# fuxiao0719/PanopticNeRF

Hardware: AMD Instinct MI355X
Metric: Msamples/sec (coarse+fine), KITTI-360 1408x376 (higher is better)
Workload: dtype bf16

## Files before the change

include/pnr.h:

```cpp
#ifndef PNR_H
#define PNR_H
#include <stdint.h>

#ifdef __cplusplus
extern "C" {
#endif

#define PNR_OK 0
#define PNR_EINVAL (-1)
#define PNR_EHIP (-2)
#define PNR_ENODEV (-3)

#define PNR_PREC_BF16 0
#define PNR_PREC_FP32 1

int pnr_version(void);
const char* pnr_last_error(void);
int pnr_device_check(int dev, char* buf_host, int buflen);

int pnr_stratified(const float* rays, int64_t n_rays, int n_samples, int lindisp,
                   const float* t_rand, float* z_out, void* stream);

int pnr_points(const float* rays, const float* z, int64_t n_rays, int n_samples, float* pts_out,
               void* stream);

int pnr_embed(const float* x, int64_t n, int L, float* out, void* stream);

typedef struct pnr_mlp_desc {
    int32_t D, W, skip;
    int32_t xyz_L, dir_L;
    int32_t n_sem, n_inst, head_W;
    int32_t precision;
    int32_t plan;
    int32_t head_tap;
    int32_t head_depth;
    int32_t schedule;
    int32_t clk_probe[2];
    int32_t flags;
} pnr_mlp_desc;

#define PNR_MLP_SOFTMAX 1
#define PNR_MLP_WG_CAP(n) (((n) & 0x1FF) << 16)
#define PNR_MLP_TRACE 0x7A00

typedef struct pnr_mlp_params_host {
    const float* const* pts_w; const float* const* pts_b;
    const float* alpha_w; const float* alpha_b;
    const float* feature_w; const float* feature_b;
    const float* views_w; const float* views_b;
    const float* rgb_w; const float* rgb_b;
    const float* sem0_w; const float* sem0_b; const float* sem1_w; const float* sem1_b;
    const float* inst0_w; const float* inst0_b; const float* inst1_w; const float* inst1_b;
} pnr_mlp_params_host;

int64_t pnr_mlp_packed_bytes(const pnr_mlp_desc* desc);
int pnr_mlp_pack(const pnr_mlp_desc* desc, const pnr_mlp_params_host* params, void* packed_host);

int64_t pnr_mlp_pack_workspace_bytes(const pnr_mlp_desc* desc, int backward);
int pnr_mlp_pack_device(const pnr_mlp_desc* desc, const pnr_mlp_params_host* params_dev, int backward,
                        void* workspace, void* packed, void* stream);
int pnr_mlp_repack_device(const pnr_mlp_desc* desc, const pnr_mlp_params_host* params_dev, int backward,
                          void* workspace, void* packed, void* stream);

int pnr_mlp_forward(const pnr_mlp_desc* desc, const void* packed, const float* rays, const float* z,
                    int64_t n_rays, int n_samples, float* raw, int64_t raw_stride_s,
                    int64_t raw_stride_c, void* stream);

int pnr_mlp_fused_plan(const pnr_mlp_desc* desc);
int64_t pnr_mlp_forward_composite_workspace_bytes(const pnr_mlp_desc* desc, int64_t n_rays, int n_samples, int want_weights);
int pnr_mlp_forward_composite(const pnr_mlp_desc* desc, const void* packed, const float* rays, const float* z,
                              int64_t n_rays, int n_samples, const int32_t* label_sem, const int32_t* label_inst,
                              int white_bkgd, float* rgb, float* depth, float* acc, float* weights, float* sem,
                              float* inst, float* fix_sem, float* fix_inst, void* workspace, void* stream);

int pnr_mlp_forward_tiles(const pnr_mlp_desc* desc, const void* packed, const float* rays, const float* z, int64_t n_rays,
                          int n_samples, void* workspace, void* stream);
int pnr_composite_combine(const pnr_mlp_desc* desc, const void* workspace, const float* z, int64_t n_rays, int n_samples,
                          const int32_t* label_sem, const int32_t* label_inst, int white_bkgd, float* rgb, float* depth,
                          float* acc, float* weights, float* sem, float* inst, float* fix_sem, float* fix_inst, void* stream);

int pnr_mlp_query(const pnr_mlp_desc* desc, const void* packed, const float* points, int64_t n_points,
                  float* sigma, int32_t* sem_label, int32_t* inst_label, int32_t* panoptic, const int32_t* is_thing,
                  float* sem_logits, float* inst_logits, int64_t logit_stride, void* stream);
int pnr_mlp_query_supported(const pnr_mlp_desc* desc);

int pnr_mlp_train_layout(const pnr_mlp_desc* desc, int64_t n_samples, int64_t* acts_off_host ,
                         int64_t* dys_off_host );
int pnr_mlp_forward_train(const pnr_mlp_desc* desc, const void* packed, const float* rays, const float* z,
                          int64_t n_rays, int n_samples, float* raw, int64_t raw_stride_s,
                          int64_t raw_stride_c, void* acts, void* stream);
int64_t pnr_mlp_bwd_packed_bytes(const pnr_mlp_desc* desc);
int pnr_mlp_pack_bwd(const pnr_mlp_desc* desc, const pnr_mlp_params_host* params, void* packed_host);
int pnr_mlp_backward(const pnr_mlp_desc* desc, const void* packed_bwd, const float* d_raw, const void* acts,
                     void* dys, int64_t n_rays, int n_samples, void* stream);

int64_t pnr_mlp_wgrad_workspace_bytes(const pnr_mlp_desc* desc, int64_t n_samples);
int pnr_mlp_wgrad(const pnr_mlp_desc* desc, const void* acts, const void* dys, int64_t n_samples,
                  const pnr_mlp_params_host* grads_dev, void* workspace, void* stream);

int64_t pnr_mlp_fp32_acts_floats(const pnr_mlp_desc* desc, int64_t n_samples);
int64_t pnr_mlp_backward_fp32_workspace_bytes(const pnr_mlp_desc* desc, int64_t n_samples);
int pnr_mlp_forward_train_fp32(const pnr_mlp_desc* desc, const pnr_mlp_params_host* params_dev, const float* rays,
                               const float* z, int64_t n_rays, int n_samples, float* raw, int64_t raw_stride_s,
                               int64_t raw_stride_c, float* acts, void* stream);
int pnr_mlp_backward_fp32(const pnr_mlp_desc* desc, const pnr_mlp_params_host* params_dev, const float* d_raw,
                          int64_t d_raw_stride_c, const float* acts, int64_t n_rays, int n_samples,
                          const pnr_mlp_params_host* grads_dev, void* workspace, void* stream);

int pnr_composite(const float* raw, int64_t raw_stride_s, int64_t raw_stride_c, const float* z,
                  const float* rays, const float* noise, const int32_t* label_sem,
                  const int32_t* label_inst, int64_t n_rays, int n_samples, int n_sem, int n_inst,
                  int sem_mode, int white_bkgd, float* rgb, float* depth, float* acc, float* weights,
                  float* sem, float* inst, float* fix_sem, float* fix_inst, void* stream);

int pnr_composite_backward(const float* raw, int64_t raw_stride_c, const float* z, const float* rays,
                           const float* noise, int64_t n_rays, int n_samples, int n_sem, int n_inst,
                           const float* g_rgb, const float* g_depth, const float* g_acc, const float* g_sem,
                           const float* g_inst, const float* g_weights, float* d_raw, void* stream);

int pnr_composite_backward2(const float* raw, int64_t raw_stride_c, const float* z, const float* rays,
                            const float* noise, int64_t n_rays, int n_samples, int n_sem, int n_inst,
                            const float* g_rgb, const float* g_depth, const float* g_acc, const float* g_sem,
                            const float* g_inst, const float* g_weights, const int32_t* label_sem,
                            const int32_t* label_inst, const float* g_fix_sem, const float* g_fix_inst,
                            const float* ce_sem, const float* ce_inst, float* d_raw, void* stream);
int pnr_composite_backward3(const float* raw, int64_t raw_stride_c, const float* z, const float* rays,
                            const float* noise, int64_t n_rays, int n_samples, int n_sem, int n_inst, int sem_mode,
                            const float* g_rgb, const float* g_depth, const float* g_acc, const float* g_sem,
                            const float* g_inst, const float* g_weights, const int32_t* label_sem,
                            const int32_t* label_inst, const float* g_fix_sem, const float* g_fix_inst,
                            const float* ce_sem, const float* ce_inst, float* d_raw, void* stream);

typedef struct pnr_loss_cfg {
    float w_rgb, w_depth, w_sem, w_fix_sem, w_inst, w_fix_inst;
    int32_t depth_l2;
    float fix_eps;
    int32_t maps_are_prob;
} pnr_loss_cfg;
int64_t pnr_losses_workspace_bytes(int64_t n_rays);
int pnr_losses(const pnr_loss_cfg* cfg, int64_t n_rays, int n_sem, int n_inst, const float* rgb, const float* depth,
               const float* sem, const float* fix_sem, const float* inst, const float* fix_inst, const float* rgb_gt,
               const float* depth_gt, const int32_t* sem_gt, const int32_t* inst_gt, float* losses_out, float* g_rgb,
               float* g_depth, float* g_sem, float* g_fix_sem, float* g_inst, float* g_fix_inst, void* workspace, void* stream);

int64_t pnr_ce3d_workspace_bytes(int64_t n_samples);
int pnr_ce3d(const float* raw, int64_t raw_stride_c, int first_channel, int n_classes, const int32_t* label,
             int64_t n_samples, float* out2, void* workspace, void* stream);

int pnr_gen_rays(const float* intr4_host, const float* c2w12_host, int width, int height, float near_, float far_,
                 const int32_t* pix, int64_t n_rays, float* rays, void* stream);

#define PNR_FISHEYE_NEWTON_STEPS 8
#define PNR_CAMERA_PINHOLE 0
#define PNR_CAMERA_FISHEYE 1

int pnr_gen_rays_fisheye(const float* cam7_host, const float* c2w12_host, int width, int height, float near_, float far_,
                         const int32_t* pix, int64_t n_rays, float* rays, uint8_t* valid, void* stream);

int pnr_project_points(int model, const float* cam_host, const float* w2c12_host, int width, int height, const float* points,
                       int64_t n, float* uv, float* range, uint8_t* valid, void* stream);

int pnr_panoptic_labels(const float* sem, const float* inst, const int32_t* is_thing, int64_t n_rays, int n_sem, int n_inst,
// ... 60 lines not shown
```

panopticnerf_amd/_lib.py:

```python
import ctypes
import os

_HERE = os.path.dirname(os.path.abspath(__file__))
LIB_PATH = os.environ.get("PNR_LIB_PATH") or os.path.join(_HERE, "libpnr.so")

c_f = ctypes.c_void_p
c_i64 = ctypes.c_int64
c_int = ctypes.c_int

PREC_BF16, PREC_FP32 = 0, 1
MLP_SOFTMAX, MLP_TRACE = 1, 0x7A00
CAMERA_PINHOLE, CAMERA_FISHEYE = 0, 1


class LossCfg(ctypes.Structure):
    _fields_ = [("w_rgb", ctypes.c_float), ("w_depth", ctypes.c_float), ("w_sem", ctypes.c_float),
                ("w_fix_sem", ctypes.c_float), ("w_inst", ctypes.c_float), ("w_fix_inst", ctypes.c_float),
                ("depth_l2", ctypes.c_int32), ("fix_eps", ctypes.c_float), ("maps_are_prob", ctypes.c_int32)]


class MlpDesc(ctypes.Structure):
    _fields_ = [("D", ctypes.c_int32), ("W", ctypes.c_int32), ("skip", ctypes.c_int32),
                ("xyz_L", ctypes.c_int32), ("dir_L", ctypes.c_int32),
                ("n_sem", ctypes.c_int32), ("n_inst", ctypes.c_int32), ("head_W", ctypes.c_int32),
                ("precision", ctypes.c_int32), ("plan", ctypes.c_int32), ("head_tap", ctypes.c_int32),
                ("head_depth", ctypes.c_int32), ("schedule", ctypes.c_int32), ("clk_probe", ctypes.c_int32 * 2), ("flags", ctypes.c_int32)]


class RngDesc(ctypes.Structure):
    _fields_ = [("call", ctypes.c_void_p), ("ray_base", ctypes.c_int64), ("tag", ctypes.c_int32), ("scale", ctypes.c_float)]


_fp = ctypes.POINTER(ctypes.c_float)
_fpp = ctypes.POINTER(_fp)


class MlpParamsHost(ctypes.Structure):
    _fields_ = [("pts_w", _fpp), ("pts_b", _fpp),
                ("alpha_w", _fp), ("alpha_b", _fp), ("feature_w", _fp), ("feature_b", _fp),
                ("views_w", _fp), ("views_b", _fp), ("rgb_w", _fp), ("rgb_b", _fp),
                ("sem0_w", _fp), ("sem0_b", _fp), ("sem1_w", _fp), ("sem1_b", _fp),
                ("inst0_w", _fp), ("inst0_b", _fp), ("inst1_w", _fp), ("inst1_b", _fp)]


SIGNATURES = {
    "pnr_version": (c_int, []),
    "pnr_last_error": (ctypes.c_char_p, []),
    "pnr_device_check": (c_int, [c_int, ctypes.c_char_p, c_int]),
    "pnr_stratified": (c_int, [c_f, c_i64, c_int, c_int, c_f, c_f, c_f]),
    "pnr_points": (c_int, [c_f, c_f, c_i64, c_int, c_f, c_f]),
    "pnr_embed": (c_int, [c_f, c_i64, c_int, c_f, c_f]),
    "pnr_mlp_packed_bytes": (c_i64, [ctypes.POINTER(MlpDesc)]),
    "pnr_mlp_pack": (c_int, [ctypes.POINTER(MlpDesc), ctypes.POINTER(MlpParamsHost), ctypes.c_void_p]),
    "pnr_mlp_pack_workspace_bytes": (c_i64, [ctypes.POINTER(MlpDesc), c_int]),
    "pnr_mlp_pack_device": (c_int, [ctypes.POINTER(MlpDesc), ctypes.POINTER(MlpParamsHost), c_int, c_f, c_f, c_f]),
    "pnr_mlp_repack_device": (c_int, [ctypes.POINTER(MlpDesc), ctypes.POINTER(MlpParamsHost), c_int, c_f, c_f, c_f]),
    "pnr_mlp_forward": (c_int, [ctypes.POINTER(MlpDesc), c_f, c_f, c_f, c_i64, c_int, c_f, c_i64, c_i64, c_f]),
    "pnr_mlp_train_layout": (c_int, [ctypes.POINTER(MlpDesc), c_i64, ctypes.POINTER(c_i64), ctypes.POINTER(c_i64)]),
    "pnr_mlp_forward_train": (c_int, [ctypes.POINTER(MlpDesc), c_f, c_f, c_f, c_i64, c_int, c_f, c_i64, c_i64, c_f, c_f]),
    "pnr_mlp_bwd_packed_bytes": (c_i64, [ctypes.POINTER(MlpDesc)]),
    "pnr_mlp_pack_bwd": (c_int, [ctypes.POINTER(MlpDesc), ctypes.POINTER(MlpParamsHost), ctypes.c_void_p]),
    "pnr_mlp_backward": (c_int, [ctypes.POINTER(MlpDesc), c_f, c_f, c_f, c_f, c_i64, c_int, c_f]),
    "pnr_mlp_wgrad_workspace_bytes": (c_i64, [ctypes.POINTER(MlpDesc), c_i64]),
    "pnr_mlp_wgrad": (c_int, [ctypes.POINTER(MlpDesc), c_f, c_f, c_i64, ctypes.POINTER(MlpParamsHost), c_f, c_f]),
    "pnr_mlp_fp32_acts_floats": (c_i64, [ctypes.POINTER(MlpDesc), c_i64]),
    "pnr_mlp_backward_fp32_workspace_bytes": (c_i64, [ctypes.POINTER(MlpDesc), c_i64]),
    "pnr_mlp_forward_train_fp32": (c_int, [ctypes.POINTER(MlpDesc), ctypes.POINTER(MlpParamsHost), c_f, c_f, c_i64, c_int, c_f, c_i64,
                                           c_i64, c_f, c_f]),
    "pnr_mlp_backward_fp32": (c_int, [ctypes.POINTER(MlpDesc), ctypes.POINTER(MlpParamsHost), c_f, c_i64, c_f, c_i64, c_int,
                                      ctypes.POINTER(MlpParamsHost), c_f, c_f]),
    "pnr_mlp_fused_plan": (c_int, [ctypes.POINTER(MlpDesc)]),
    "pnr_mlp_forward_composite_workspace_bytes": (c_i64, [ctypes.POINTER(MlpDesc), c_i64, c_int, c_int]),
    "pnr_mlp_forward_composite": (c_int, [ctypes.POINTER(MlpDesc), c_f, c_f, c_f, c_i64, c_int, c_f, c_f, c_int,
                                          c_f, c_f, c_f, c_f, c_f, c_f, c_f, c_f, c_f, c_f]),
    "pnr_composite": (c_int, [c_f, c_i64, c_i64, c_f, c_f, c_f, c_f, c_f, c_i64, c_int, c_int, c_int, c_int,
                              c_int, c_f, c_f, c_f, c_f, c_f, c_f, c_f, c_f, c_f]),
    "pnr_composite_backward": (c_int, [c_f, c_i64, c_f, c_f, c_f, c_i64, c_int, c_int, c_int,
                                       c_f, c_f, c_f, c_f, c_f, c_f, c_f, c_f]),
    "pnr_composite_backward2": (c_int, [c_f, c_i64, c_f, c_f, c_f, c_i64, c_int, c_int, c_int,
                                        c_f, c_f, c_f, c_f, c_f, c_f, c_f, c_f, c_f, c_f, c_f, c_f, c_f, c_f]),
    "pnr_composite_backward3": (c_int, [c_f, c_i64, c_f, c_f, c_f, c_i64, c_int, c_int, c_int, c_int,
                                        c_f, c_f, c_f, c_f, c_f, c_f, c_f, c_f, c_f, c_f, c_f, c_f, c_f, c_f]),
    "pnr_losses_workspace_bytes": (c_i64, [c_i64]),
    "pnr_losses": (c_int, [ctypes.POINTER(LossCfg), c_i64, c_int, c_int] + [c_f] * 19),
    "pnr_ce3d_workspace_bytes": (c_i64, [c_i64]),
    "pnr_ce3d": (c_int, [c_f, c_i64, c_int, c_int, c_f, c_i64, c_f, c_f, c_f]),
    "pnr_gen_rays": (c_int, [ctypes.POINTER(ctypes.c_float), ctypes.POINTER(ctypes.c_float), c_int, c_int, ctypes.c_float,
                             ctypes.c_float, c_f, c_i64, c_f, c_f]),
    "pnr_gen_rays_fisheye": (c_int, [ctypes.POINTER(ctypes.c_float), ctypes.POINTER(ctypes.c_float), c_int, c_int, ctypes.c_float,
                                     ctypes.c_float, c_f, c_i64, c_f, c_f, c_f]),
    "pnr_project_points": (c_int, [c_int, ctypes.POINTER(ctypes.c_float), ctypes.POINTER(ctypes.c_float), c_int, c_int, c_f, c_i64,
                                   c_f, c_f, c_f, c_f]),
    "pnr_panoptic_labels": (c_int, [c_f, c_f, c_f, c_i64, c_int, c_int, c_f, c_f, c_f, c_f]),
    "pnr_confusion": (c_int, [c_f, c_f, c_i64, c_int, c_f, c_f]),
    "pnr_sample_pdf": (c_int, [c_f, c_f, c_f, c_i64, c_int, c_int, c_f, c_f, c_f, c_f]),
    "pnr_bbox_hits": (c_int, [c_f, c_i64, c_f, c_int, c_int, c_f, c_f, c_f, c_f]),
    "pnr_restrict_rays": (c_int, [c_f, c_i64, c_f, c_f, c_int, c_f, c_f]),
    "pnr_sample_labels": (c_int, [c_f, c_i64, c_int, c_f, c_f, c_f, c_int, c_f, c_f, c_f, c_f]),
    "pnr_ray_setup": (c_int, [c_f, c_i64, c_f, c_int, c_int, c_f, c_int, c_int, c_f, c_int, c_f, c_f, c_f, c_f, c_f, c_f, c_f]),
    "pnr_sample_pdf_labels": (c_int, [c_f, c_f, c_f, c_i64, c_int, c_int, c_f, c_f, c_f, c_f, c_int, c_f, c_f, c_f, c_f]),
    "pnr_mlp_forward_tiles": (c_int, [ctypes.POINTER(MlpDesc), c_f, c_f, c_f, c_i64, c_int, c_f, c_f]),
    "pnr_rng_begin": (c_int, [c_f, c_f, c_f]),
    "pnr_rng_fill": (c_int, [ctypes.POINTER(RngDesc), c_i64, c_int, c_int, c_f, c_f]),
    "pnr_stratified_rng": (c_int, [c_f, c_i64, c_int, c_int, ctypes.POINTER(RngDesc), c_f, c_f]),
    "pnr_ray_setup_rng": (c_int, [c_f, c_i64, c_f, c_int, c_int, c_f, c_int, c_int, ctypes.POINTER(RngDesc), c_int, c_f, c_f, c_f, c_f,
                                  c_f, c_f, c_f]),
    "pnr_sample_pdf_rng": (c_int, [c_f, c_f, ctypes.POINTER(RngDesc), c_i64, c_int, c_int, c_f, c_f, c_f, c_f]),
    "pnr_sample_pdf_labels_rng": (c_int, [c_f, c_f, ctypes.POINTER(RngDesc), c_i64, c_int, c_int, c_f, c_f, c_f, c_f, c_int, c_f, c_f, c_f,
                                          c_f]),
    "pnr_composite_rng": (c_int, [c_f, c_i64, c_i64, c_f, c_f, ctypes.POINTER(RngDesc), c_f, c_f, c_i64, c_int, c_int, c_int, c_int,
                                  c_int, c_f, c_f, c_f, c_f, c_f, c_f, c_f, c_f, c_f]),
    "pnr_composite_backward_rng": (c_int, [c_f, c_i64, c_f, c_f, ctypes.POINTER(RngDesc), c_i64, c_int, c_int, c_int, c_int,
                                           c_f, c_f, c_f, c_f, c_f, c_f, c_f, c_f, c_f, c_f, c_f, c_f, c_f, c_f]),
    "pnr_mlp_query": (c_int, [ctypes.POINTER(MlpDesc), c_f, c_f, c_i64, c_f, c_f, c_f, c_f, c_f, c_f, c_f, c_i64, c_f]),
    "pnr_mlp_query_supported": (c_int, [ctypes.POINTER(MlpDesc)]),
    "pnr_composite_combine": (c_int, [ctypes.POINTER(MlpDesc), c_f, c_f, c_i64, c_int, c_f, c_f, c_int,
                                      c_f, c_f, c_f, c_f, c_f, c_f, c_f, c_f, c_f]),
}

_lib = None


def load():
    global _lib
    if _lib is not None:
        return _lib
    if not os.path.exists(LIB_PATH):
        raise RuntimeError(
            f"{LIB_PATH} not found: the HIP extension is not built. Run "
            "`python -c 'import __graft_entry__ as g; g.build()'` (or `make -C panopticnerf_amd/csrc`). "
            "There is no CPU fallback.")
    lib = ctypes.CDLL(LIB_PATH)
    for name, (res, args) in SIGNATURES.items():
        fn = getattr(lib, name)
        fn.restype = res
        fn.argtypes = args
    _lib = lib
    return lib


def check(rc, what):
    if rc != 0:
        msg = load().pnr_last_error().decode(errors="replace")
        raise RuntimeError(f"{what} failed (code {rc}): {msg}")
```

panopticnerf_amd/csrc/pnr_composite.hip:

```cpp
#include <stdlib.h>

#include "pnr_common.h"
#include "pnr_fuse_record.h"
#include "pnr_lane_ops.h"
#include "pnr_philox.h"

struct CompositeArgs {
    const float* raw; int64_t stride_s, stride_c;
    const float* z; const float* rays; const float* noise;
    const int32_t* label_sem; const int32_t* label_inst;
    int64_t R; int N, C, K, sem_mode, white_bkgd;
    float *rgb, *depth, *acc, *weights, *sem, *inst, *fix_sem, *fix_inst;
    int use_hist;
};

struct f4 { float v[4]; };
#ifndef CMP_GRID_PER_CU
#define CMP_GRID_PER_CU 8
#endif
#ifndef CMP_UB
#define CMP_UB 8
#endif
#define CMP_FIX_SCALE 1073741824.0f
#ifndef CMP_PREFETCH
#define CMP_PREFETCH 0
#endif

template <bool CH_MAJOR>
__device__ __forceinline__ f4 load4(const float* __restrict__ raw, int64_t ss, int64_t sc, int64_t s0, int c, bool active)
{
    f4 o;
    if (!active) { o.v[0] = o.v[1] = o.v[2] = o.v[3] = 0.0f; return o; }
    if (CH_MAJOR) {
        const float4 t = *reinterpret_cast<const float4*>(raw + (int64_t)c * sc + s0);
        o.v[0] = t.x; o.v[1] = t.y; o.v[2] = t.z; o.v[3] = t.w;
    } else {
        const float* p = raw + s0 * ss + (int64_t)c * sc;
#pragma unroll
        for (int k = 0; k < 4; ++k) o.v[k] = p[k * ss];
    }
    return o;
}

__device__ __forceinline__ float dot4(const f4& w, const f4& v)
{
    return fmaf(w.v[3], v.v[3], fmaf(w.v[2], v.v[2], fmaf(w.v[1], v.v[1], w.v[0] * v.v[0])));
}

template <bool CH_MAJOR, int SUB, bool SOFTMAX, class... Rng>
__global__ __launch_bounds__(256) void k_composite(CompositeArgs a, const Rng... rng)
{
    constexpr bool RNG = sizeof...(Rng) > 0;
    extern __shared__ __attribute__((aligned(16))) uint32_t s_hist[];
    constexpr int RPW = 64 / SUB;
    const int lane = threadIdx.x & 63, wave = threadIdx.x >> 6;
    const int N = a.N, nq4 = N >> 2;
    const int q = lane & (SUB - 1);
    const int g = lane / SUB;
    const int64_t wave_global = ((int64_t)blockIdx.x * blockDim.x + threadIdx.x) >> 6;
    const int64_t n_waves = ((int64_t)gridDim.x * blockDim.x) >> 6;
    const int64_t n_groups = (a.R + RPW - 1) / RPW;
    const int CK = a.C + a.K;
    const int nq = 3 + CK;
    uint32_t* hist = s_hist + ((size_t)wave * RPW + g) * CK;
    PnrRngKey key;
    if constexpr (RNG) key = pnr_rng_key(rng...);

    auto load_zs = [&](int64_t grp, f4& zz, f4& sg) {
        const int64_t ray = grp * RPW + g;
        const bool active = (ray < a.R) && (q < nq4) && (grp < n_groups);
        const int64_t rayc = ray < a.R ? ray : a.R - 1;
        const int64_t s0 = rayc * N + (active ? 4 * q : 0);
        if (active) {
            const float4 t = *reinterpret_cast<const float4*>(a.z + s0);
            zz.v[0] = t.x; zz.v[1] = t.y; zz.v[2] = t.z; zz.v[3] = t.w;
        } else {
            zz.v[0] = zz.v[1] = zz.v[2] = zz.v[3] = 0.0f;
        }
        sg = load4<CH_MAJOR>(a.raw, a.stride_s, a.stride_c, s0, 3, active);
    };
    f4 pz, ps;
    if (CMP_PREFETCH) load_zs(wave_global, pz, ps);

    for (int64_t grp = wave_global; grp < n_groups; grp += n_waves) {
// ... 387 lines not shown

static int composite_impl(const float* raw, int64_t raw_stride_s, int64_t raw_stride_c, const float* z, const float* rays,
                          const float* noise, const PnrRngDev* rng, const int32_t* label_sem, const int32_t* label_inst, int64_t n_rays,
                          int n_samples, int n_sem, int n_inst, int sem_mode, int white_bkgd, float* rgb, float* depth, float* acc,
                          float* weights, float* sem, float* inst, float* fix_sem, float* fix_inst, void* stream);

PNR_EXPORT int pnr_composite(const float* raw, int64_t raw_stride_s, int64_t raw_stride_c, const float* z,
                             const float* rays, const float* noise, const int32_t* label_sem,
                             const int32_t* label_inst, int64_t n_rays, int n_samples, int n_sem, int n_inst,
                             int sem_mode, int white_bkgd, float* rgb, float* depth, float* acc, float* weights,
                             float* sem, float* inst, float* fix_sem, float* fix_inst, void* stream)
{
    return composite_impl(raw, raw_stride_s, raw_stride_c, z, rays, noise, nullptr, label_sem, label_inst, n_rays, n_samples, n_sem, n_inst,
                          sem_mode, white_bkgd, rgb, depth, acc, weights, sem, inst, fix_sem, fix_inst, stream);
}

PNR_EXPORT int pnr_composite_rng(const float* raw, int64_t raw_stride_s, int64_t raw_stride_c, const float* z, const float* rays,
                                 const pnr_rng* noise_host, const int32_t* label_sem, const int32_t* label_inst, int64_t n_rays,
                                 int n_samples, int n_sem, int n_inst, int sem_mode, int white_bkgd, float* rgb, float* depth, float* acc,
                                 float* weights, float* sem, float* inst, float* fix_sem, float* fix_inst, void* stream)
{
    PnrRngDev rng;
    const int rc = pnr_rng_check(noise_host, n_rays < 0 ? 0 : n_rays, "pnr_composite_rng", &rng);
    if (rc) return rc;
    PNR_REQUIRE(n_rays <= 0 || (raw_stride_s == 1 && (raw_stride_c % 4) == 0 && (((uintptr_t)raw) & 15) == 0),
                "pnr_composite_rng: channel-major, 16-byte aligned raw images only");
    return composite_impl(raw, raw_stride_s, raw_stride_c, z, rays, nullptr, &rng, label_sem, label_inst, n_rays, n_samples, n_sem, n_inst,
                          sem_mode, white_bkgd, rgb, depth, acc, weights, sem, inst, fix_sem, fix_inst, stream);
}

static int composite_impl(const float* raw, int64_t raw_stride_s, int64_t raw_stride_c, const float* z, const float* rays,
                          const float* noise, const PnrRngDev* rng, const int32_t* label_sem, const int32_t* label_inst, int64_t n_rays,
                          int n_samples, int n_sem, int n_inst, int sem_mode, int white_bkgd, float* rgb, float* depth, float* acc,
                          float* weights, float* sem, float* inst, float* fix_sem, float* fix_inst, void* stream)
{
    PNR_REQUIRE(n_rays <= 0 || (raw && z && rays), "pnr_composite: null pointer");
    PNR_REQUIRE(n_samples >= 4 && n_samples <= 256 && (n_samples % 4) == 0,
                "pnr_composite: n_samples=%d must be a multiple of 4 in [4,256]", n_samples);
    PNR_REQUIRE(n_sem >= 0 && n_inst >= 0 && (sem_mode == 0 || sem_mode == 1), "pnr_composite: bad field sizes");
    PNR_REQUIRE((((uintptr_t)z) & 15) == 0, "pnr_composite: z must be 16-byte aligned");
    PNR_REQUIRE(!weights || (((uintptr_t)weights) & 15) == 0, "pnr_composite: weights must be 16-byte aligned");
    PNR_REQUIRE((((uintptr_t)noise) & 15) == 0 && (((uintptr_t)label_sem) & 15) == 0 && (((uintptr_t)label_inst) & 15) == 0,
                "pnr_composite: noise / label arrays must be 16-byte aligned");
    if (n_rays <= 0) return PNR_OK;
    CompositeArgs a;
    a.raw = raw; a.stride_s = raw_stride_s; a.stride_c = raw_stride_c; a.z = z; a.rays = rays; a.noise = noise;
    a.label_sem = label_sem; a.label_inst = label_inst; a.R = n_rays; a.N = n_samples; a.C = n_sem; a.K = n_inst;
    a.sem_mode = sem_mode; a.white_bkgd = white_bkgd; a.rgb = rgb; a.depth = depth; a.acc = acc; a.weights = weights;
    a.sem = sem; a.inst = inst; a.fix_sem = fix_sem; a.fix_inst = fix_inst;
    int sub = 1;
    while (sub < n_samples / 4) sub <<= 1;
    const int rpw = 64 / sub;
    const size_t hist_bytes = (size_t)4 * rpw * (n_sem + n_inst) * sizeof(uint32_t);
    const bool want_fix = (fix_sem && label_sem && n_sem) || (fix_inst && label_inst && n_inst);
    a.use_hist = (want_fix && hist_bytes <= 48 * 1024) ? 1 : 0;
    const size_t lds = a.use_hist ? hist_bytes : 0;
    const bool ch_major = raw_stride_s == 1 && (raw_stride_c % 4) == 0 && (((uintptr_t)raw) & 15) == 0;
    hipStream_t st = (hipStream_t)stream;
    const int variant = composite_variant();
    if (ch_major && n_samples > 32 && ((variant >= 1 && n_samples <= 64) || variant >= 2)) {
        const int L = n_samples > 64 ? 16 : 8;
        const int m4 = (n_samples + 4 * L - 1) / (4 * L);
        const int rpw2 = 64 / L;
        const size_t hb = (size_t)4 * rpw2 * (n_sem + n_inst) * sizeof(uint32_t);
        if (!want_fix || hb <= 48 * 1024) {
            const int64_t ng = (n_rays + rpw2 - 1) / rpw2;
            const int grid2 = pnr_grid_cap((ng + 3) / 4, CMP_GRID_PER_CU);
            a.use_hist = want_fix ? 1 : 0;
            if (sem_mode) launch_composite2<true>(L, m4, grid2, want_fix ? hb : 0, st, a, rng); else launch_composite2<false>(L, m4, grid2, want_fix ? hb : 0, st, a, rng);
            PNR_CHECK_LAUNCH("pnr_composite");
            return PNR_OK;
        }
    }
    const int64_t n_groups = (n_rays + rpw - 1) / rpw;
    const int grid = pnr_grid_cap((n_groups + 3) / 4, CMP_GRID_PER_CU);
    if (rng) { if (sem_mode) launch_composite_rng<true>(sub, grid, lds, st, a, *rng); else launch_composite_rng<false>(sub, grid, lds, st, a, *rng); }
    else if (ch_major) { if (sem_mode) launch_composite<true, true>(sub, grid, lds, st, a); else launch_composite<true, false>(sub, grid, lds, st, a); }
    else { if (sem_mode) launch_composite<false, true>(sub, grid, lds, st, a); else launch_composite<false, false>(sub, grid, lds, st, a); }
    PNR_CHECK_LAUNCH("pnr_composite");
    return PNR_OK;
}


struct CombineArgs {
    const float* rec; int rec_floats; const float4* ps; const float* z; const int32_t* lab_s; const int32_t* lab_i;
    int64_t R; int N, C, K, white_bkgd;
    float *rgb, *depth, *acc, *weights, *sem, *inst, *fix_sem, *fix_inst;
};

template <bool LOGITS>
__global__ __launch_bounds__(256) void k_composite_combine(CombineArgs a)
{
    __shared__ uint32_t hist_all[4][128];
    const int lane = threadIdx.x & 63, wv = threadIdx.x >> 6;
    const int64_t ray = ((int64_t)blockIdx.x * blockDim.x + threadIdx.x) >> 6;
    if (ray >= a.R) return;
    const int N = a.N, T = N >> 5, RF = a.rec_floats, C = a.C, K = a.K, CK = C + K;
    const float* __restrict__ rec = a.rec + ray * T * RF;
    const float4* __restrict__ ps = a.ps + ray * N;
    const float* __restrict__ zr = a.z + ray * N;
    const bool want_s = a.lab_s && a.fix_sem && C, want_i = a.lab_i && a.fix_inst && K;
    const int32_t* __restrict__ lsr = want_s ? a.lab_s + ray * N : nullptr;
    const int32_t* __restrict__ lir = want_i ? a.lab_i + ray * N : nullptr;
    float q[8];
#pragma unroll
    for (int k = 0; k < 8; ++k) q[k] = k < T ? rec[k * RF] : 1.0f;
    float4 pv[4];
    float zv[4];
    int lsv[4], liv[4];
#pragma unroll
    for (int j = 0; j < 4; ++j) {
        const int i = lane + 64 * j;
        const bool in = i < N;
        pv[j] = in ? ps[i] : float4{0.0f, 0.0f, 0.0f, 0.0f};
        zv[j] = in ? zr[i] : 0.0f;
        lsv[j] = (in && want_s) ? lsr[i] : -1;
        liv[j] = (in && want_i) ? lir[i] : -1;
    }
    float lg[2][8];
#pragma unroll
    for (int h = 0; h < 2; ++h)
#pragma unroll
        for (int k = 0; k < 8; ++k) lg[h][k] = (LOGITS && k < T && lane + 64 * h < CK) ? rec[k * RF + PNR_FUSE_REC_LOGITS + lane + 64 * h] : 0.0f;
    float Tk[8];
    float t = 1.0f;
#pragma unroll
    for (int k = 0; k < 8; ++k) {
        Tk[k] = t;
        if (k < T) t *= q[k];
    }
    uint32_t* hist = hist_all[wv];
    if (want_s || want_i)
        for (int c = lane; c < CK; c += 64) hist[c] = 0;
    float r5[5] = {0.0f, 0.0f, 0.0f, 0.0f, 0.0f};
#pragma unroll
    for (int j = 0; j < 4; ++j) {
        const int i = lane + 64 * j;
        if (i < N) {
            const float4 p = pv[j];
            float tk = Tk[0];
#pragma unroll
            for (int k = 1; k < 8; ++k) tk = (i >> 5) == k ? Tk[k] : tk;
            const float w = tk * p.x;
            r5[0] += w;
            r5[1] = fmaf(w, zv[j], r5[1]);
            r5[2] = fmaf(w, 1.0f / (1.0f + expf(-p.y)), r5[2]);
            r5[3] = fmaf(w, 1.0f / (1.0f + expf(-p.z)), r5[3]);
            r5[4] = fmaf(w, 1.0f / (1.0f + expf(-p.w)), r5[4]);
            if (a.weights) a.weights[ray * N + i] = w;
            if (want_s || want_i) {
                const uint32_t fx = (uint32_t)(w * PNR_FUSE_FIX_SCALE + 0.5f);
                if (want_s) { const int l = lsv[j]; if (l >= 0 && l < C) atomicAdd(&hist[l], fx); }
                if (want_i) { const int l = liv[j]; if (l >= 0 && l < K) atomicAdd(&hist[C + l], fx); }
            }
        }
    }
    group_sum_batch<64, 5>(r5);
    if (lane == 0) {
        if (a.acc) a.acc[ray] = r5[0];
        if (a.depth) a.depth[ray] = r5[1];
    }
    if (lane < 3 && a.rgb) {
        const float v = lane == 0 ? r5[2] : lane == 1 ? r5[3] : r5[4];
        a.rgb[ray * 3 + lane] = a.white_bkgd ? v + (1.0f - r5[0]) : v;
    }
#pragma unroll
    for (int h = 0; h < 2; ++h) {
        const int c = lane + 64 * h;
        if (c >= CK) continue;
        if constexpr (LOGITS) {
            float v = 0.0f;
#pragma unroll
            for (int k = 0; k < 8; ++k) if (k < T) v = fmaf(Tk[k], lg[h][k], v);
            if (c < C) { if (a.sem) a.sem[ray * C + c] = v; }
            else if (a.inst) a.inst[ray * K + (c - C)] = v;
        }
        if (c < C) { if (want_s) a.fix_sem[ray * C + c] = (float)hist[c] * (1.0f / PNR_FUSE_FIX_SCALE); }
        else if (want_i) a.fix_inst[ray * K + (c - C)] = (float)hist[c] * (1.0f / PNR_FUSE_FIX_SCALE);
    }
}

int pnr_composite_combine_launch(const float* rec, int rec_floats, bool logit_sums, const float4* ps, const float* z,
                                 const int32_t* label_sem, const int32_t* label_inst, int64_t R, int N, int C, int K, int white_bkgd,
                                 float* rgb, float* depth, float* acc, float* weights, float* sem, float* inst, float* fix_sem,
                                 float* fix_inst, hipStream_t st)
{
    CombineArgs a;
    a.rec = rec; a.rec_floats = rec_floats; a.ps = ps; a.z = z; a.lab_s = label_sem; a.lab_i = label_inst;
    a.R = R; a.N = N; a.C = C; a.K = K; a.white_bkgd = white_bkgd;
    a.rgb = rgb; a.depth = depth; a.acc = acc; a.weights = weights; a.sem = sem; a.inst = inst; a.fix_sem = fix_sem; a.fix_inst = fix_inst;
    const int64_t blocks = (R + 3) / 4;
    if (logit_sums) hipLaunchKernelGGL(k_composite_combine<true>, dim3((unsigned)blocks), dim3(256), 0, st, a);
    else hipLaunchKernelGGL(k_composite_combine<false>, dim3((unsigned)blocks), dim3(256), 0, st, a);
    PNR_CHECK_LAUNCH("pnr_mlp_forward_composite (combine)");
    return PNR_OK;
}
```

panopticnerf_amd/csrc/pnr_mlp.hip:

```cpp
#include <stdlib.h>
#include <string.h>

#include "pnr_mlp_plan.h"

int pnr_mlp_validate(const pnr_mlp_desc* d);

#include "pnr_mlp_core.h"
#include "pnr_mlp_pp.h"
#ifndef PNR_FUSE_TRANSPOSED
#define PNR_FUSE_TRANSPOSED 1
#endif
#include "pnr_mlp_fuse.h"
#include "pnr_mlp_tt.h"
#define PNR_QUERY_MAX_POINTS (((int64_t)1 << 31) - 4096)
#ifndef PNR_TRAIN_TILES_EXPERIMENT
#define PNR_TRAIN_TILES_EXPERIMENT 0
#endif
template <int PREC, int TILES, class CTX, int KIND, int NA, int NB, int NFB_OUT, int MODE, int NOUT>
__device__ __forceinline__ void layer_regs(CTX& c, const uint32_t (&inA)[TILES][NA],
                                           const uint32_t (&inB)[TILES][NB > 0 ? NB : 1],
                                           uint32_t (&out)[TILES][NOUT], uint16_t* save = nullptr,
                                           const int* srow = nullptr)
{
    constexpr int RPB = PrecT<PREC>::RPB;
// ... 718 lines not shown
}


static inline unsigned long long* clk_probe_of(const pnr_mlp_desc* d)
{
    return (unsigned long long*)(uintptr_t)(((uint64_t)(uint32_t)d->clk_probe[1] << 32) | (uint64_t)(uint32_t)d->clk_probe[0]);
}

static void mlp_args_fill(MlpArgs& a, const pnr_mlp_desc* desc, const PnrPlan& plan, const void* packed)
{
    memset(&a, 0, sizeof(a));
    a.data = (const uint8_t*)packed + plan.data_off;
    a.table = (const pnr_chunk_entry*)((const uint8_t*)packed + plan.table_off);
    a.n_chunks = (int)plan.chunks.size();
    a.slot_bytes = plan.max_chunk_frags * PNR_FRAG_BYTES;
    a.D = desc->D; a.skip = desc->skip; a.n_sem = desc->n_sem; a.n_inst = desc->n_inst;
    a.head_tap = desc->head_tap; a.head_depth = desc->head_depth == 1 ? 1 : 2;
    a.clk = clk_probe_of(desc);
#if PNR_TRACE
    if (const char* e = getenv("PNR_TRACE_PTR")) a.trace = (unsigned long long*)strtoull(e, nullptr, 0);
#endif
}

static int mlp_forward_impl(const pnr_mlp_desc* desc, const void* packed, const float* rays, const float* z,
                            int64_t n_rays, int n_samples, float* raw, int64_t raw_stride_s, int64_t raw_stride_c,
                            void* acts, void* stream)
{
    int rc = pnr_mlp_validate(desc);
    if (rc != PNR_OK) return rc;
    PNR_REQUIRE(n_rays >= 0 && n_samples >= 1, "pnr_mlp_forward: bad size");
    if (n_rays == 0) return PNR_OK;
    PNR_REQUIRE(packed && rays && z && raw, "pnr_mlp_forward: null pointer");
    PNR_REQUIRE(n_rays * (int64_t)n_samples < ((int64_t)1 << 31) - 4096, "pnr_mlp_forward: R*N=%lld exceeds 2^31",
                (long long)(n_rays * n_samples));
    PNR_REQUIRE((((uintptr_t)rays) & 15) == 0 && (((uintptr_t)packed) & 15) == 0 && (((uintptr_t)acts) & 15) == 0,
                "pnr_mlp_forward: rays / packed / acts must be 16-byte aligned");
    PNR_REQUIRE(!acts || desc->precision == PNR_PREC_BF16, "pnr_mlp_forward_train: the training path is bf16 only");
    PNR_REQUIRE(desc->plan != 4, "pnr_mlp_forward: a plan-4 (field) image is for pnr_mlp_query only");
    PNR_REQUIRE(desc->plan == 0, "pnr_mlp_forward: plan=%d images are for pnr_mlp_forward_composite only", desc->plan);
    PnrPlan plan;
    pnr_build_plan(*desc, plan);
    MlpArgs a;
    mlp_args_fill(a, desc, plan, packed);
    a.rays = rays; a.z = z; a.S = (int)(n_rays * n_samples); a.N = n_samples;
    pnr_set_div_magic(n_samples, a.n_magic, a.n_shift);
    a.raw = raw; a.ss = raw_stride_s; a.sc = raw_stride_c;
    a.acts = (uint16_t*)acts;
    if (acts) pnr_train_layout(*desc, a.S, a.acts_off, a.dys_off, a.gate_off);
    hipStream_t st = (hipStream_t)stream;
    if (desc->precision == PNR_PREC_BF16) {
        if (desc->schedule != 1 && !acts)
            return desc->W == 256 ? launch_mlp_pp<256, false>(a, st) : launch_mlp_pp<128, false>(a, st);
        if (desc->schedule == 2 && acts)
            return desc->W == 256 ? launch_mlp_pp<256, true>(a, st) : launch_mlp_pp<128, true>(a, st);
#if PNR_TRAIN_TILES_EXPERIMENT
        if (acts && desc->schedule == 3 && desc->W == 256) return launch_mlp<PNR_PREC_BF16, 256, 2, 4, 1, true>(a, st);
        if (acts && desc->schedule == 4 && desc->W == 256) {
            PNR_REQUIRE(a.S % 384 == 0, "schedule 4 (experiment): S must be a multiple of 384");
            return launch_mlp<PNR_PREC_BF16, 256, 3, 4, 1, true>(a, st);
        }
#endif
        if (acts)
            return desc->W == 256 ? launch_mlp<PNR_PREC_BF16, 256, 1, 8, 2, true>(a, st)
                                  : launch_mlp<PNR_PREC_BF16, 128, 1, 8, 2, true>(a, st);
        return desc->W == 256 ? launch_mlp<PNR_PREC_BF16, 256, 1, 8, 2>(a, st) : launch_mlp<PNR_PREC_BF16, 128, 1, 8, 2>(a, st);
    }
    return desc->W == 256 ? launch_mlp<PNR_PREC_FP32, 256, 1, 4, 1>(a, st) : launch_mlp<PNR_PREC_FP32, 128, 1, 4, 1>(a, st);
}

PNR_EXPORT int pnr_mlp_forward(const pnr_mlp_desc* desc, const void* packed, const float* rays, const float* z,
                               int64_t n_rays, int n_samples, float* raw, int64_t raw_stride_s,
                               int64_t raw_stride_c, void* stream)
{
    return mlp_forward_impl(desc, packed, rays, z, n_rays, n_samples, raw, raw_stride_s, raw_stride_c, nullptr, stream);
}

#define PNR_RAY_AUX_BYTES 128
#define PNR_TT_SAVE_REGION (352 * 1024)
static bool pnr_tt_save_proto() { static const bool on = getenv("PNR_TT_SAVE_PROTO") != nullptr; return on; }
int pnr_composite_combine_launch(const float* rec, int rec_floats, bool logit_sums, const float4* ps, const float* z,
                                 const int32_t* label_sem, const int32_t* label_inst, int64_t R, int N, int C, int K, int white_bkgd,
                                 float* rgb, float* depth, float* acc, float* weights, float* sem, float* inst, float* fix_sem,
                                 float* fix_inst, hipStream_t st);

static int record_floats(const pnr_mlp_desc& d)
{
    return d.plan == 3 ? pnr_fuse_record_floats(0, 0) : pnr_fuse_record_floats(d.n_sem, d.n_inst);
}

PNR_EXPORT int64_t pnr_mlp_forward_composite_workspace_bytes(const pnr_mlp_desc* desc, int64_t n_rays, int n_samples, int want_weights)
{
    (void)want_weights;
    if (pnr_mlp_validate(desc) != PNR_OK || n_rays < 0 || n_samples < 32 || (n_samples & 31)) return -1;
    const int64_t S = n_rays * n_samples, tiles = (S + 255) / 256 * 8;
    if (desc->plan == 3) return tiles * record_floats(*desc) * 4 + S * 16 + 256;
    return tiles * pnr_fuse_record_floats(desc->n_sem, desc->n_inst) * 4 + S * 16 + 256 + PNR_RAY_AUX_BYTES + n_rays * PNR_RAY_AUX_BYTES +
           (pnr_tt_save_proto() ? tiles / 8 * 4 * PNR_TT_SAVE_REGION + 4096 : 0);
}

__global__ void __launch_bounds__(256) k_ray_aux(const float* __restrict__ rays, int64_t R, uint32_t* __restrict__ aux)
{
    const int64_t i = (int64_t)blockIdx.x * 256 + threadIdx.x;
    if (i >= 2 * R) return;
    const int64_t ray = i >> 1;
    const int hi = (int)(i & 1);
    const float dx = rays[ray * 8 + 3], dy = rays[ray * 8 + 4], dz = rays[ray * 8 + 5];
    const float nrm = sqrtf(__fadd_rn(__fadd_rn(__fmul_rn(dx, dx), __fmul_rn(dy, dy)), __fmul_rn(dz, dz)));
    uint32_t ed[8];
    embed_lane<PNR_PREC_BF16, 2, 16, 8>(dx / nrm, dy / nrm, dz / nrm, hi, ed);
    uint4* o = reinterpret_cast<uint4*>(aux + i * 16);
    o[0] = make_uint4(ed[0], ed[1], ed[2], ed[3]);
    o[1] = make_uint4(ed[4], ed[5], ed[6], ed[7]);
    o[2] = make_uint4(__float_as_uint(nrm), 0u, 0u, 0u);
}

static int fused_mlp_launch(const pnr_mlp_desc* desc, const void* packed, const float* rays, const float* z, int64_t n_rays,
                            int n_samples, void* workspace, void* stream, MlpArgs& a)
{
    int rc = pnr_mlp_validate(desc);
    if (rc != PNR_OK) return rc;
    PNR_REQUIRE(desc->precision == PNR_PREC_BF16, "pnr_mlp_forward_composite: bf16 only");
    PNR_REQUIRE(desc->plan != 4, "pnr_mlp_forward_composite: a plan-4 (field) image is for pnr_mlp_query only");
    PNR_REQUIRE(n_rays >= 1 && n_samples >= 32 && n_samples <= 256 && (n_samples & 31) == 0,
                "pnr_mlp_forward_composite: n_samples=%d must be a multiple of 32 in [32,256]", n_samples);
    PNR_REQUIRE(desc->n_sem + desc->n_inst <= 128, "pnr_mlp_forward_composite: n_sem + n_inst <= 128");
    PNR_REQUIRE(packed && rays && z && workspace, "pnr_mlp_forward_composite: null pointer");
    PNR_REQUIRE(n_rays * (int64_t)n_samples < ((int64_t)1 << 31) - 4096, "pnr_mlp_forward_composite: R*N exceeds 2^31");
    PNR_REQUIRE((((uintptr_t)rays | (uintptr_t)packed | (uintptr_t)workspace) & 15) == 0,
                "pnr_mlp_forward_composite: rays / packed / workspace must be 16-byte aligned");
    PnrPlan plan;
    pnr_build_plan(*desc, plan);
    mlp_args_fill(a, desc, plan, packed);
    a.rays = rays; a.z = z; a.S = (int)(n_rays * n_samples); a.N = n_samples;
    pnr_set_div_magic(n_samples, a.n_magic, a.n_shift);
    a.rec_floats = record_floats(*desc);
    a.rec = (float*)workspace;
    const int64_t tiles = ((int64_t)a.S + 255) / 256 * 8;
    a.ps = (float4*)(a.rec + tiles * a.rec_floats);
    hipStream_t st = (hipStream_t)stream;
    const bool softmax = (desc->flags & PNR_MLP_SOFTMAX) && desc->n_sem + desc->n_inst > 0;
    if (desc->plan == 3)
        return desc->W == 256 ? launch_mlp_pp<256, false, true, 0, true>(a, st) : launch_mlp_pp<128, false, true, 0, true>(a, st);
    if (desc->plan == 2) {
        PnrTTArgs t;
        memset(&t, 0, sizeof(t));
        t.image = a.data; t.rays = rays; t.z = z; t.S = a.S; t.N = a.N; t.n_magic = a.n_magic; t.n_shift = a.n_shift;
        t.rec = a.rec; t.rec_floats = a.rec_floats; t.ps = a.ps; t.n_sem = a.n_sem; t.n_inst = a.n_inst; t.clk = a.clk;
        PNR_REQUIRE(n_rays < ((int64_t)1 << 24), "pnr_mlp_forward_composite: the two-tile kernel addresses 2^24 rays per launch");
        uint32_t* aux = (uint32_t*)(((uintptr_t)((uint8_t*)a.ps + (int64_t)a.S * 16 + 256) + PNR_RAY_AUX_BYTES - 1)
                                    & ~(uintptr_t)(PNR_RAY_AUX_BYTES - 1));
        k_ray_aux<<<dim3((unsigned)((2 * n_rays + 255) / 256)), dim3(256), 0, st>>>(rays, n_rays, aux);
        t.aux = aux;
        t.n_wg = (desc->flags >> 16) & 0x1FF;
        if (pnr_tt_save_proto()) t.save = (void*)(((uintptr_t)((uint8_t*)aux + n_rays * PNR_RAY_AUX_BYTES) + 4095) & ~(uintptr_t)4095);
        const bool trace = (desc->flags & 0xFF00) == PNR_MLP_TRACE;
        return pnr_mlp_tt_launch(t, (desc->n_sem + 31) / 32, (desc->n_inst + 31) / 32, a.head_depth, a.head_tap, softmax, st, trace,
                                 trace ? ((desc->flags >> 4) & 7) : 0);
    }
    if (desc->plan == 1) {
        const int nbs = (desc->n_sem + 31) / 32, nbi = (desc->n_inst + 31) / 32;
        switch (4 * nbs + nbi + (softmax ? 16 : 0)) {
        case 4: return launch_mlp_pp<256, false, true, 4>(a, st);
        case 5: return launch_mlp_pp<256, false, true, 5>(a, st);
        case 8: return launch_mlp_pp<256, false, true, 8>(a, st);
        case 9: return launch_mlp_pp<256, false, true, 9>(a, st);
        case 20: return launch_mlp_pp<256, false, true, 20>(a, st);
        case 21: return launch_mlp_pp<256, false, true, 21>(a, st);
        case 24: return launch_mlp_pp<256, false, true, 24>(a, st);
        case 25: return launch_mlp_pp<256, false, true, 25>(a, st);
        default: PNR_REQUIRE(false, "pnr_mlp_forward_composite: no plan-1 kernel for %d + %d logit blocks", nbs, nbi);
        }
    }
    PNR_REQUIRE(!softmax, "pnr_mlp_forward_composite: softmax compositing needs the plan-1 image (pnr_mlp_fused_plan >= 1, desc.plan = 1)");
    return desc->W == 256 ? launch_mlp_pp<256, false, true>(a, st) : launch_mlp_pp<128, false, true>(a, st);
}

PNR_EXPORT int pnr_mlp_forward_tiles(const pnr_mlp_desc* desc, const void* packed, const float* rays, const float* z, int64_t n_rays,
                                     int n_samples, void* workspace, void* stream)
{
    PNR_REQUIRE(n_rays >= 0, "pnr_mlp_forward_tiles: bad size");
    if (n_rays == 0) return PNR_OK;
    MlpArgs a;
    return fused_mlp_launch(desc, packed, rays, z, n_rays, n_samples, workspace, stream, a);
}

PNR_EXPORT int pnr_composite_combine(const pnr_mlp_desc* desc, const void* workspace, const float* z, int64_t n_rays, int n_samples,
                                     const int32_t* label_sem, const int32_t* label_inst, int white_bkgd, float* rgb, float* depth,
                                     float* acc, float* weights, float* sem, float* inst, float* fix_sem, float* fix_inst, void* stream)
{
    int rc = pnr_mlp_validate(desc);
    if (rc != PNR_OK) return rc;
    PNR_REQUIRE(n_rays >= 0 && n_samples >= 32 && n_samples <= 256 && (n_samples & 31) == 0, "pnr_composite_combine: bad size");
    if (n_rays == 0) return PNR_OK;
    PNR_REQUIRE(workspace && z, "pnr_composite_combine: null pointer");
    PNR_REQUIRE(desc->plan != 4, "pnr_composite_combine: a plan-4 (field) image has no compositing workspace");
    PNR_REQUIRE((!fix_sem || label_sem) && (!fix_inst || label_inst), "pnr_composite_combine: fix_* outputs need their labels");
    PNR_REQUIRE(desc->plan != 3 || (!rgb && !sem && !inst), "pnr_composite_combine: a plan-3 (sigma-only) workspace has no rgb, semantic "
                "or instance maps: pass null for them");
    const int rf = record_floats(*desc);
    const int64_t tiles = (n_rays * n_samples + 255) / 256 * 8;
    const float* rec = (const float*)workspace;
    return pnr_composite_combine_launch(rec, rf, desc->plan != 3, (const float4*)(rec + tiles * rf), z, fix_sem ? label_sem : nullptr,
                                        fix_inst ? label_inst : nullptr, n_rays, n_samples, desc->n_sem, desc->n_inst, white_bkgd,
                                        rgb, depth, acc, weights, sem, inst, fix_sem, fix_inst, (hipStream_t)stream);
}

PNR_EXPORT int pnr_mlp_forward_composite(const pnr_mlp_desc* desc, const void* packed, const float* rays, const float* z,
                                         int64_t n_rays, int n_samples, const int32_t* label_sem, const int32_t* label_inst,
                                         int white_bkgd, float* rgb, float* depth, float* acc, float* weights, float* sem,
                                         float* inst, float* fix_sem, float* fix_inst, void* workspace, void* stream)
{
    PNR_REQUIRE(n_rays >= 0, "pnr_mlp_forward_composite: bad size");
    if (n_rays == 0) return PNR_OK;
    PNR_REQUIRE((!fix_sem || label_sem) && (!fix_inst || label_inst), "pnr_mlp_forward_composite: fix_* outputs need their labels");
    PNR_REQUIRE(!desc || desc->plan != 3 || (!rgb && !sem && !inst), "pnr_mlp_forward_composite: a plan-3 (sigma-only) image has no "
                "rgb, semantic or instance maps: pass null for them");
    MlpArgs a;
    int rc = fused_mlp_launch(desc, packed, rays, z, n_rays, n_samples, workspace, stream, a);
    if (rc != PNR_OK) return rc;
    return pnr_composite_combine_launch(a.rec, a.rec_floats, desc->plan != 3, a.ps, z, fix_sem ? label_sem : nullptr, fix_inst ? label_inst : nullptr,
                                        n_rays, n_samples, desc->n_sem, desc->n_inst, white_bkgd, rgb, depth, acc, weights, sem, inst,
                                        fix_sem, fix_inst, (hipStream_t)stream);
}

PNR_EXPORT int pnr_mlp_forward_train(const pnr_mlp_desc* desc, const void* packed, const float* rays, const float* z,
                                     int64_t n_rays, int n_samples, float* raw, int64_t raw_stride_s,
                                     int64_t raw_stride_c, void* acts, void* stream)
{
    PNR_REQUIRE(acts || n_rays == 0, "pnr_mlp_forward_train: acts is null");
    return mlp_forward_impl(desc, packed, rays, z, n_rays, n_samples, raw, raw_stride_s, raw_stride_c, acts, stream);
}

PNR_EXPORT int pnr_mlp_train_layout(const pnr_mlp_desc* desc, int64_t n_samples, int64_t* acts_off_host,
                                    int64_t* dys_off_host)
{
    int rc = pnr_mlp_validate(desc);
    if (rc != PNR_OK) return rc;
    PNR_REQUIRE(acts_off_host && dys_off_host && n_samples >= 0, "pnr_mlp_train_layout: bad arguments");
    int64_t a[24], d[24];
    pnr_train_layout(*desc, n_samples, a, d);
    memcpy(acts_off_host, a, sizeof(int64_t) * (size_t)(desc->D + 7));
    memcpy(dys_off_host, d, sizeof(int64_t) * (size_t)(desc->D + 8));
    return PNR_OK;
}

struct FieldArgs {
    MlpArgs m;
    const float* pts;
    float* sigma;
    int32_t* sem_label; int32_t* inst_label; int32_t* panoptic;
    const int32_t* is_thing;
    float* sem_logits; float* inst_logits; int64_t lstride;
    int run_sem, run_inst;
};

template <class CTX, int NA, class EPI>
__device__ __forceinline__ void pp_field_out(CTX& c, u32x4 (&A)[CTX::P], const uint32_t (&in)[NA], int n_out, EPI&& epi)
{
    using CH = PPChunk<1, NA, 0>;
    const uint32_t dummy[1] = {0};
    const int nfb = (n_out + 31) >> 5;
#pragma unroll 1
    for (int fb = 0; fb < nfb; ++fb) {
        f32x16 acc[1];
        CH::prologue(c.frag_addr(), c.bias_addr(), A, acc);
        CH::mma(c.frag_addr(), A, in, dummy, acc, [&](auto... k) { if constexpr (sizeof...(k) == 0) { c.stamp(6); c.barrier(); c.stamp(2); } else c.stamp(k...); });
        c.m_done();
        c.refill_begin();
        c.refill_one();
        epi(fb, acc[0]);
        c.refill_rest();
        c.advance();
    }
}

struct FieldBest { float v; int i; };
__device__ __forceinline__ void field_best_merge(FieldBest& b, int hi)
{
    const auto pv = __builtin_amdgcn_permlane32_swap(__float_as_uint(b.v), __float_as_uint(b.v), false, false);
    const auto pi = __builtin_amdgcn_permlane32_swap((uint32_t)b.i, (uint32_t)b.i, false, false);
    const float ov = __uint_as_float(hi ? pv[0] : pv[1]);
    const int oi = (int)(hi ? pi[0] : pi[1]);
    if (ov > b.v || (ov == b.v && oi < b.i)) { b.v = ov; b.i = oi; }
    if (b.i == 0x7fffffff) b.i = 0;
}

template <int W, bool HEADS>
__global__ __launch_bounds__(512, 2) void k_mlp_pp_field(const FieldArgs fa)
{
    constexpr int WAVES = 8;
    using CTX = CtxPP<WAVES>;
    extern __shared__ __attribute__((aligned(16))) char smem[];
    constexpr int NFB = W / 32, HFB = W / 64;
    constexpr int HR = NFB * 8, GR = HFB * 8, GXR = 16;
    const MlpArgs& a = fa.m;
    CTX c = pp_ctx<WAVES>(a, smem);
    unsigned long long clk_c0, clk_r0;
    pp_begin(c, clk_c0, clk_r0);
    const int n = c.lane & 31;

    uint32_t dummy[1] = {0};
    u32x4 A[CTX::P];
    struct PointIn { float x, y, z; };
    auto fetch_point = [&](int grp) {
        const int s = (grp * WAVES + c.wave) * 32 + n;
// ... 119 lines not shown
```

panopticnerf_amd/csrc/pnr_mlp_pack.cpp:

```cpp
#include <math.h>
#include <string.h>

#include <vector>

#include "pnr_common.h"
#include "pnr_mlp_layout.h"
#include "pnr_mlp_plan.h"
#include "pnr_mlp_tt.h"

int pnr_mlp_validate(const pnr_mlp_desc* d)
{
    PNR_REQUIRE(d, "pnr_mlp: null desc");
    PNR_REQUIRE(d->W == 256 || d->W == 128, "pnr_mlp: W=%d unsupported (128 or 256)", d->W);
    PNR_REQUIRE(d->D >= 2 && d->D <= 16, "pnr_mlp: D=%d outside [2,16]", d->D);
    PNR_REQUIRE(d->skip >= -1 && d->skip < d->D - 1, "pnr_mlp: skip=%d must be -1 or < D-1", d->skip);
    PNR_REQUIRE(d->xyz_L >= 0 && d->xyz_L <= 10, "pnr_mlp: xyz_L=%d outside [0,10]", d->xyz_L);
    PNR_REQUIRE(d->dir_L >= 0 && d->dir_L <= 4, "pnr_mlp: dir_L=%d outside [0,4]", d->dir_L);
    PNR_REQUIRE(d->n_sem >= 0 && d->n_sem <= 256 && d->n_inst >= 0 && d->n_inst <= 256,
                "pnr_mlp: n_sem/n_inst outside [0,256]");
    PNR_REQUIRE((d->n_sem == 0 && d->n_inst == 0) || d->head_W == d->W / 2,
                "pnr_mlp: head_W=%d must equal W/2=%d", d->head_W, d->W / 2);
    PNR_REQUIRE(d->precision == PNR_PREC_BF16 || d->precision == PNR_PREC_FP32, "pnr_mlp: bad precision %d",
                d->precision);
    PNR_REQUIRE(d->head_tap == 0 || d->head_tap == 1, "pnr_mlp: head_tap=%d must be 0 (trunk output) or 1 (feature)", d->head_tap);
    PNR_REQUIRE(d->head_depth >= 0 && d->head_depth <= 2, "pnr_mlp: head_depth=%d must be 1 or 2", d->head_depth);
#ifndef PNR_TRAIN_TILES_EXPERIMENT
#define PNR_TRAIN_TILES_EXPERIMENT 0
#endif
    PNR_REQUIRE(d->schedule >= 0 && d->schedule <= (PNR_TRAIN_TILES_EXPERIMENT ? 6 : 2), "pnr_mlp: schedule=%d must be 0 (default), 1 (lock-step) or 2 (ping-pong)", d->schedule);
    PNR_REQUIRE(d->plan == 0 || (d->plan == 1 && pnr_plan1_supported(*d)) || (d->plan == 2 && pnr_plan2_supported(*d)) ||
                (d->plan == 3 && pnr_plan3_supported(*d)) || (d->plan == 4 && pnr_plan4_supported(*d)),
                "pnr_mlp: plan=%d is not available for this geometry (ask pnr_mlp_fused_plan; plans 3 and 4: bf16 only)", d->plan);
    const uint32_t trace = (uint32_t)d->flags & 0xFF00u;
    PNR_REQUIRE(((uint32_t)d->flags & ~(uint32_t)(PNR_MLP_SOFTMAX | 0xFF70u | PNR_MLP_WG_CAP(0x1FF))) == 0 && (trace == 0 || trace == PNR_MLP_TRACE) &&
                (trace != 0 || ((uint32_t)d->flags & 0x70u) == 0),
                "pnr_mlp: unknown bits in flags=0x%x (zero-initialise pnr_mlp_desc; PNR_MLP_* are the defined bits)", (unsigned)d->flags);
    PNR_REQUIRE(((uint32_t)d->clk_probe[0] & 15u) == 0, "pnr_mlp: clk_probe=0x%08x%08x is not a 16-byte aligned device address "
                "(zero-initialise pnr_mlp_desc; clk_probe is a diagnostics field, 0 = off)", (unsigned)d->clk_probe[1], (unsigned)d->clk_probe[0]);
    PNR_REQUIRE(trace == 0 || (d->clk_probe[0] | d->clk_probe[1]) != 0, "pnr_mlp: PNR_MLP_TRACE needs clk_probe");
    return PNR_OK;
}

PNR_EXPORT int pnr_mlp_fused_plan(const pnr_mlp_desc* desc)
{
    if (!desc) return 0;
    pnr_mlp_desc d = *desc;
    d.plan = 0;
    if (pnr_mlp_validate(&d) != PNR_OK) return 0;
    if ((d.flags & PNR_MLP_SOFTMAX) && d.n_sem + d.n_inst > 0)
        return pnr_plan2_supported(d) ? 2 : pnr_plan1_supported(d) ? 1 : 0;
    return pnr_plan2_supported(d) ? 2 : pnr_plan1_supported(d) ? 1 : 0;
}

PNR_EXPORT int pnr_mlp_query_supported(const pnr_mlp_desc* desc)
{
    if (!desc) return 0;
    pnr_mlp_desc d = *desc;
    d.plan = 0;
    if (pnr_mlp_validate(&d) != PNR_OK) return 0;
    return pnr_plan4_supported(d);
}

static int bwd_validate(const pnr_mlp_desc* d)
{
    int rc = pnr_mlp_validate(d);
    if (rc != PNR_OK) return rc;
    PNR_REQUIRE(d->plan == 0, "pnr_mlp backward: plan must be 0");
    PNR_REQUIRE(d->precision == PNR_PREC_BF16, "pnr_mlp backward: bf16 only");
    PNR_REQUIRE(d->n_sem <= PNR_BWD_OUT_SLOTS && d->n_inst <= PNR_BWD_OUT_SLOTS,
                "pnr_mlp backward: n_sem / n_inst must be <= %d", PNR_BWD_OUT_SLOTS);
    return PNR_OK;
}

static int check_params(const pnr_mlp_desc* desc, const pnr_mlp_params_host* p, bool bias)
{
    PNR_REQUIRE(p, "pnr_mlp_pack: null params");
    if (desc->plan == 3) {
        PNR_REQUIRE(p->pts_w && p->alpha_w && (!bias || (p->pts_b && p->alpha_b)), "pnr_mlp_pack: missing trunk or alpha_linear parameter");
        return PNR_OK;
    }
    if (desc->plan == 4) {
        const bool feat = desc->head_tap == 1 && (desc->n_sem || desc->n_inst);
        PNR_REQUIRE(p->pts_w && p->alpha_w && (!bias || (p->pts_b && p->alpha_b)), "pnr_mlp_pack: missing trunk or alpha_linear parameter");
        PNR_REQUIRE(!feat || (p->feature_w && (!bias || p->feature_b)), "pnr_mlp_pack: missing feature_linear parameter");
    } else {
    PNR_REQUIRE(p->pts_w && p->alpha_w && p->feature_w && p->views_w && p->rgb_w, "pnr_mlp_pack: missing trunk parameter");
    if (bias) PNR_REQUIRE(p->pts_b && p->alpha_b && p->feature_b && p->views_b && p->rgb_b, "pnr_mlp_pack: missing trunk bias");
    }
    const bool deep = pnr_head_depth(*desc) == 2;
    if (desc->n_sem) PNR_REQUIRE((!deep || p->sem0_w) && p->sem1_w && (!bias || ((!deep || p->sem0_b) && p->sem1_b)), "pnr_mlp_pack: missing semantic head");
    if (desc->n_inst) PNR_REQUIRE((!deep || p->inst0_w) && p->inst1_w && (!bias || ((!deep || p->inst0_b) && p->inst1_b)), "pnr_mlp_pack: missing instance head");
    return PNR_OK;
}

struct Image {
    pnr_pack_header hdr;
    std::vector<pnr_chunk_entry> table;
    std::vector<PnrFragDesc> frags;
    size_t table_off, data_off, total_bytes;
};

static PnrFragDesc zero_desc()
{
    PnrFragDesc f;
    memset(&f, 0, sizeof(f));
    return f;
}

static void fill_header(Image& im, const pnr_mlp_desc& d, int version, size_t n_chunks, int max_frags, size_t table_off,
                        size_t data_off, size_t total)
{
    memset(&im.hdr, 0, sizeof(im.hdr));
    im.hdr.magic = PNR_PACK_MAGIC;
    im.hdr.version = (uint32_t)version;
    im.hdr.n_chunks = (uint32_t)n_chunks;
    im.hdr.max_chunk_frags = (uint32_t)max_frags;
    im.hdr.table_off = (uint32_t)table_off;
// ... 273 lines not shown
```

panopticnerf_amd/csrc/pnr_sampling.hip:

```cpp
#include "pnr_common.h"
#include "pnr_philox.h"
#include <stdlib.h>
#include <string.h>

#pragma clang fp contract(off)

__device__ __forceinline__ float pnr_linspace01(int i, int N)
{
    if (N <= 1) return 0.0f;
    const float step = 1.0f / (float)(N - 1);
    if (i < N / 2) return step * (float)i;
    return fmaf(-step, (float)(N - 1 - i), 1.0f);
}

__device__ __forceinline__ float strat_z(float nr, float fr, int i, int N, int lindisp)
{
    const float t = pnr_linspace01(i, N);
    const float omt = 1.0f - t;
    if (!lindisp) {
        const float a = nr * omt, b = fr * t;
        return a + b;
    }
    const float a = (1.0f / nr) * omt, b = (1.0f / fr) * t;
    return 1.0f / (a + b);
}

__device__ __forceinline__ float strat_sample(float nr, float fr, int i, int N, int lindisp, const float* t)
{
    const float zi = strat_z(nr, fr, i, N, lindisp);
    if (!t) return zi;
    const float z0 = strat_z(nr, fr, 0, N, lindisp), zl = strat_z(nr, fr, N - 1, N, lindisp);
    const float lo = (i == 0) ? z0 : 0.5f * (zi + strat_z(nr, fr, i - 1, N, lindisp));
    const float up = (i == N - 1) ? zl : 0.5f * (strat_z(nr, fr, i + 1, N, lindisp) + zi);
    const float w = up - lo;
    const float m = w * *t;
    return lo + m;
}

struct GenRaysArgs { float fx, fy, cx, cy; float c2w[12]; int width; float near_, far_; const int32_t* pix; int64_t R; float* rays; };
__global__ __launch_bounds__(256) void k_gen_rays(const GenRaysArgs a)
{
    for (int64_t r = (int64_t)blockIdx.x * blockDim.x + threadIdx.x; r < a.R; r += (int64_t)gridDim.x * blockDim.x) {
        const int64_t p = a.pix ? (int64_t)a.pix[r] : r;
        const int j = (int)(p / a.width), i = (int)(p - (int64_t)j * a.width);
        const float x = ((float)i - a.cx) / a.fx;
        const float y = ((float)j - a.cy) / a.fy;
        float d[3];
#pragma unroll
        for (int k = 0; k < 3; ++k) {
            const float u = a.c2w[k * 4 + 0] * x, v = a.c2w[k * 4 + 1] * y;
            d[k] = (u + v) + a.c2w[k * 4 + 2];
        }
        float4* o = reinterpret_cast<float4*>(a.rays + r * 8);
        o[0] = make_float4(a.c2w[3], a.c2w[7], a.c2w[11], d[0]);
        o[1] = make_float4(d[1], d[2], a.near_, a.far_);
    }
}

template <class... Rng>
__global__ __launch_bounds__(256) void k_stratified(const float* __restrict__ rays, int64_t R, int N,
                                                     int lindisp, const float* __restrict__ t_rand,
                                                     float* __restrict__ z_out, const Rng... rng)
{
    constexpr bool RNG = sizeof...(Rng) > 0;
    PnrRngKey key;
    if constexpr (RNG) key = pnr_rng_key(rng...);
    const int64_t total = R * N;
    for (int64_t s = (int64_t)blockIdx.x * blockDim.x + threadIdx.x; s < total;
         s += (int64_t)gridDim.x * blockDim.x) {
        const int64_t r = s / N;
        const int i = (int)(s - r * N);
        if constexpr (RNG) {
            const float t = pnr_rng_uniform_at(key, (uint32_t)r, i);
            z_out[s] = strat_sample(rays[r * 8 + 6], rays[r * 8 + 7], i, N, lindisp, &t);
        } else {
            z_out[s] = strat_sample(rays[r * 8 + 6], rays[r * 8 + 7], i, N, lindisp, t_rand ? t_rand + s : nullptr);
        }
    }
}

__global__ __launch_bounds__(256) void k_points(const float* __restrict__ rays, const float* __restrict__ z,
                                                 int64_t R, int N, float* __restrict__ pts)
// ... 161 lines not shown
            const float m = t * span;
            const float zs = s_bins[below] + m;
            if (zs_out) zs_out[r * Nf + i] = zs;
            if (inds_out) inds_out[r * Nf + i] = inds;
            s_sort[Nc + i] = zs;
        }
        if (zfine_out) {
            __syncthreads();
            bool asc = true;
            for (int i = lane; i + 1 < Nf; i += 64) asc = asc && (s_sort[Nc + i] <= s_sort[Nc + i + 1]);
            for (int i = lane; i + 1 < Nc; i += 64) asc = asc && (s_z[i] <= s_z[i + 1]);
            if (__all(asc)) {
                for (int i = lane; i < Nc; i += 64) {
                    const float v = s_z[i];
                    int lo = 0, hi = Nf;
                    while (lo < hi) { const int mid = (lo + hi) >> 1; if (s_sort[Nc + mid] < v) lo = mid + 1; else hi = mid; }
                    s_out[i + lo] = v;
                }
                for (int j = lane; j < Nf; j += 64) {
                    const float v = s_sort[Nc + j];
                    int lo = 0, hi = Nc;
                    while (lo < hi) { const int mid = (lo + hi) >> 1; if (s_z[mid] <= v) lo = mid + 1; else hi = mid; }
                    s_out[j + lo] = v;
                }
                __syncthreads();
                for (int i = lane; i < Nt; i += 64) zfine_out[r * Nt + i] = s_out[i];
                labels(r, s_out);
                __syncthreads();
                continue;
            }
            for (int i = lane; i < Nc; i += 64) s_sort[i] = s_z[i];
            for (int i = Nt + lane; i < P; i += 64) s_sort[i] = INFINITY;
            __syncthreads();
            for (int k = 2; k <= P; k <<= 1) {
                for (int j = k >> 1; j > 0; j >>= 1) {
                    for (int t = lane; t < (P >> 1); t += 64) {
                        const int i = ((t & ~(j - 1)) << 1) | (t & (j - 1));
                        const int p = i | j;
                        const float a = s_sort[i], b = s_sort[p];
                        const bool asc = (i & k) == 0;
                        if ((a > b) == asc) {
                            s_sort[i] = b;
                            s_sort[p] = a;
                        }
                    }
                    __syncthreads();
                }
            }
            for (int i = lane; i < Nt; i += 64) zfine_out[r * Nt + i] = s_sort[i];
            labels(r, s_sort);
        }
        __syncthreads();
    }
}

__device__ __noinline__ void pdf_bitonic_fallback(float* s_sort, const float* s_z, const float* s_zs, int Nc, int Nf, int P, int lane)
{
    const int Nt = Nc + Nf;
    for (int i = lane; i < Nc; i += 64) s_sort[i] = s_z[i];
    for (int i = lane; i < Nf; i += 64) s_sort[Nc + i] = s_zs[i];
    for (int i = Nt + lane; i < P; i += 64) s_sort[i] = INFINITY;
    __syncthreads();
    for (int k = 2; k <= P; k <<= 1) {
        for (int j = k >> 1; j > 0; j >>= 1) {
            for (int t = lane; t < (P >> 1); t += 64) {
                const int i = ((t & ~(j - 1)) << 1) | (t & (j - 1));
                const int p = i | j;
                const float a = s_sort[i], b = s_sort[p];
                const bool asc = (i & k) == 0;
                if ((a > b) == asc) {
                    s_sort[i] = b;
                    s_sort[p] = a;
                }
            }
            __syncthreads();
        }
    }
}

#ifndef PDF_DET_WPE
#define PDF_DET_WPE 8
#endif
#if PDF_DET_WPE
__attribute__((amdgpu_waves_per_eu(PDF_DET_WPE, PDF_DET_WPE)))
#endif
__global__ __launch_bounds__(64) void k_sample_pdf_det(const float* __restrict__ z, const float* __restrict__ weights, int64_t R, int Nc,
                                                        int Nf, float* __restrict__ zfine_out, const PdfLabelArgs lab)
{
    __shared__ float s_z[64], s_w[64], s_pdf[64], s_cdf[64], s_bins[64];
    __shared__ float s_zs[192], s_out[256];
    __shared__ float s_total, s_part[32];
    const int lane = threadIdx.x;
    const int nb = Nc - 1, nw = Nc - 2, Nt = Nc + Nf;
    int topc = 1, topf = 1;
    while (topc * 2 <= Nc) topc *= 2;
    while (topf * 2 <= Nf) topf *= 2;
    const int mh = lab.max_hits;
    for (int64_t r = blockIdx.x; r < R; r += gridDim.x) {
        const float* __restrict__ zr = z + r * Nc;
        const float* __restrict__ wr = weights + r * Nc;
        const float zl = lane < Nc ? zr[lane] : 0.0f, wl = lane < Nc ? wr[lane] : 0.0f;
        int cnt = 0, h_ls = -1, h_li = -1;
        float h_ti = 0.0f, h_to = 0.0f;
        if (lab.label_sem) {
            const int c0 = lab.hit_count[r];
            cnt = c0 < mh ? c0 : mh;
            if (lane < cnt) {
                const float2 t2 = *reinterpret_cast<const float2*>(lab.hit_t + (r * mh + lane) * 2);
                h_ti = t2.x; h_to = t2.y;
                const int m = lab.hit_box[r * mh + lane];
                h_ls = lab.box_ids[m * 2];
                h_li = lab.box_ids[m * 2 + 1];
            }
        }
        s_z[lane] = zl;
        s_w[lane] = wl;
        const float zn = __shfl_down(zl, 1, 64), wn = __shfl_down(wl, 1, 64);
        s_bins[lane] = 0.5f * (zn + zl);
        __syncthreads();
        if (lane < 32) {
            const int k = lane >> 3, l = lane & 7, nv = nw / 8, groups = nv / 4;
            float pacc = 0.0f;
            for (int g = 0; g < groups; ++g) pacc = pacc + (s_w[(g * 4 + k) * 8 + l + 1] + 1e-5f);
            if (k == 0)
                for (int v = groups * 4; v < nv; ++v) pacc = pacc + (s_w[v * 8 + l + 1] + 1e-5f);
            s_part[lane] = pacc;
        }
        __syncthreads();
        if (lane == 0) {
            const int nv = nw / 8;
            float total = 0.0f;
            for (int j = nv * 8; j < nw; ++j) total = total + (s_w[j + 1] + 1e-5f);
            for (int l = 0; l < 8; ++l) {
                float p0 = s_part[l];
                p0 = p0 + s_part[8 + l]; p0 = p0 + s_part[16 + l]; p0 = p0 + s_part[24 + l];
                total = total + p0;
            }
            s_total = total;
        }
        __syncthreads();
        const float total = s_total;
        const float pl = lane < nw ? (wn + 1e-5f) / total : 0.0f;
        s_pdf[lane] = pl;
        double c = (double)pl;
        bool exact = __all(pl == 0.0f || pl >= 0x1p-28f);
        if (exact) {
#pragma unroll
            for (int d = 1; d < 64; d <<= 1) {
                const double o = __shfl_up(c, d, 64);
                if (lane >= d) c += o;
            }
            exact = __shfl(c, 63, 64) < 1.999;
        }
        if (exact) {
            if (lane == 0) s_cdf[0] = 0.0f;
            if (lane < nw) s_cdf[lane + 1] = (float)c;
        } else {
            __syncthreads();
            if (lane == 0) {
                double cc = 0.0;
                s_cdf[0] = 0.0f;
                for (int j = 0; j < nw; ++j) {
                    cc += (double)s_pdf[j];
                    s_cdf[j + 1] = (float)cc;
                }
            }
        }
        __syncthreads();
        bool asc = lane + 1 >= Nc || zl <= zn;
        for (int i = lane; i < Nf; i += 64) {
            const float uu = pnr_linspace01(i, Nf);
            int pos = 0;
            for (int st = topc; st >= 1; st >>= 1) {
                const int p = pos + st, q = p <= nb ? p : nb;
                pos = (p <= nb && s_cdf[q - 1] <= uu) ? p : pos;
            }
            const int inds = pos;
            const int below = inds - 1 > 0 ? inds - 1 : 0;
            const int above = inds < nb - 1 ? inds : nb - 1;
            const float cb = s_cdf[below];
            float denom = s_cdf[above] - cb;
            if (denom < 1e-5f) denom = 1.0f;
            const float t = (uu - cb) / denom;
            const float bb = s_bins[below];
            const float span = s_bins[above] - bb;
            const float m = t * span;
            const float zs = bb + m;
            s_zs[i] = zs;
        }
        __syncthreads();
        for (int i = lane; i + 1 < Nf; i += 64) asc = asc && (s_zs[i] <= s_zs[i + 1]);
        if (__all(asc)) {
            if (lane < Nc) {
                int pos = 0;
                for (int st = topf; st >= 1; st >>= 1) {
                    const int p = pos + st, q = p <= Nf ? p : Nf;
                    pos = (p <= Nf && s_zs[q - 1] < zl) ? p : pos;
                }
                s_out[lane + pos] = zl;
            }
            for (int j = lane; j < Nf; j += 64) {
                const float v = s_zs[j];
                int pos = 0;
                for (int st = topc; st >= 1; st >>= 1) {
                    const int p = pos + st, q = p <= Nc ? p : Nc;
                    pos = (p <= Nc && s_z[q - 1] <= v) ? p : pos;
                }
                s_out[j + pos] = v;
            }
            __syncthreads();
        } else {
            int P = 1;
            while (P < Nt) P <<= 1;
            pdf_bitonic_fallback(s_out, s_z, s_zs, Nc, Nf, P, lane);
        }
        float* __restrict__ zo = zfine_out + r * Nt;
        for (int i0 = 0; i0 < Nt; i0 += 256) {
            float zz[4];
            int best[4], ls[4], li[4];
            float bt[4];
#pragma unroll
            for (int k = 0; k < 4; ++k) {
                const int i = i0 + lane + 64 * k;
                zz[k] = i < Nt ? s_out[i < Nt ? i : 0] : 0.0f;
                best[k] = -1; ls[k] = -1; li[k] = -1; bt[k] = 0.0f;
                if (i < Nt) zo[i] = zz[k];
            }
            if (lab.label_sem) {
                for (int h = 0; h < cnt; ++h) {
                    const float ti = __int_as_float(__builtin_amdgcn_readlane(__float_as_int(h_ti), h));
                    const float to = __int_as_float(__builtin_amdgcn_readlane(__float_as_int(h_to), h));
                    const int hs = __builtin_amdgcn_readlane(h_ls, h), hi2 = __builtin_amdgcn_readlane(h_li, h);
#pragma unroll
                    for (int k = 0; k < 4; ++k) {
                        const bool take = ti <= zz[k] && zz[k] <= to && (best[k] < 0 || ti < bt[k]);
                        best[k] = take ? h : best[k];
                        bt[k] = take ? ti : bt[k];
                        ls[k] = take ? hs : ls[k];
                        li[k] = take ? hi2 : li[k];
                    }
                }
#pragma unroll
                for (int k = 0; k < 4; ++k) {
                    const int i = i0 + lane + 64 * k;
                    if (i < Nt) {
                        lab.label_sem[r * Nt + i] = ls[k];
                        lab.label_inst[r * Nt + i] = li[k];
                    }
                }
            }
        }
        __syncthreads();
    }
}

__global__ __launch_bounds__(64) __attribute__((amdgpu_waves_per_eu(8, 8)))
void k_sample_pdf(const float* __restrict__ z, const float* __restrict__ weights, const float* __restrict__ u, int64_t R, int Nc, int Nf,
                  float* __restrict__ zs_out, int32_t* __restrict__ inds_out, float* __restrict__ zfine_out, const PdfLabelArgs lab)
{
    sample_pdf_body<64, 256>(z, weights, u, R, Nc, Nf, zs_out, inds_out, zfine_out, lab);
}
__global__ __launch_bounds__(64)
void k_sample_pdf_big(const float* __restrict__ z, const float* __restrict__ weights, const float* __restrict__ u, int64_t R, int Nc, int Nf,
                      float* __restrict__ zs_out, int32_t* __restrict__ inds_out, float* __restrict__ zfine_out, const PdfLabelArgs lab)
{
    sample_pdf_body<PDF_MAXC, PDF_MAXT>(z, weights, u, R, Nc, Nf, zs_out, inds_out, zfine_out, lab);
}
__global__ __launch_bounds__(64) __attribute__((amdgpu_waves_per_eu(8, 8)))
void k_sample_pdf_rng(const float* __restrict__ z, const float* __restrict__ weights, int64_t R, int Nc, int Nf, float* __restrict__ zs_out,
                      int32_t* __restrict__ inds_out, float* __restrict__ zfine_out, const PdfLabelArgs lab, const PnrRngDev rng)
{
    sample_pdf_body<64, 256, true>(z, weights, nullptr, R, Nc, Nf, zs_out, inds_out, zfine_out, lab, rng);
}
__global__ __launch_bounds__(64)
void k_sample_pdf_big_rng(const float* __restrict__ z, const float* __restrict__ weights, int64_t R, int Nc, int Nf,
                          float* __restrict__ zs_out, int32_t* __restrict__ inds_out, float* __restrict__ zfine_out, const PdfLabelArgs lab,
                          const PnrRngDev rng)
{
    sample_pdf_body<PDF_MAXC, PDF_MAXT, true>(z, weights, nullptr, R, Nc, Nf, zs_out, inds_out, zfine_out, lab, rng);
}

__global__ __launch_bounds__(256) void k_bbox_hits(const float* __restrict__ rays, int64_t R,
                                                    const float* __restrict__ box, int M, int max_hits,
                                                    float* __restrict__ hit_t, int32_t* __restrict__ hit_box,
                                                    int32_t* __restrict__ hit_count)
{
    for (int64_t r = (int64_t)blockIdx.x * blockDim.x + threadIdx.x; r < R;
         r += (int64_t)gridDim.x * blockDim.x) {
        const float o0 = rays[r * 8 + 0], o1 = rays[r * 8 + 1], o2 = rays[r * 8 + 2];
        const float d0 = rays[r * 8 + 3], d1 = rays[r * 8 + 4], d2 = rays[r * 8 + 5];
        const float nr = rays[r * 8 + 6], fr = rays[r * 8 + 7];
        for (int h = 0; h < max_hits; ++h) {
            hit_box[r * max_hits + h] = -1;
            hit_t[(r * max_hits + h) * 2 + 0] = 0.0f;
            hit_t[(r * max_hits + h) * 2 + 1] = 0.0f;
        }
        int cnt = 0;
        for (int m = 0; m < M; ++m) {
            const float* b = box + m * 15;
            const float p0 = o0 - b[0], p1 = o1 - b[1], p2 = o2 - b[2];
            float tmin = nr, tmax = fr;
#pragma unroll
            for (int a = 0; a < 3; ++a) {
                const float r0 = b[3 + 3 * a], r1 = b[4 + 3 * a], r2 = b[5 + 3 * a];
                const float ol = (r0 * p0 + r1 * p1) + r2 * p2;
                const float dl = (r0 * d0 + r1 * d1) + r2 * d2;
                const float inv = 1.0f / dl;
                const float e = b[12 + a];
                const float t1 = (-e - ol) * inv, t2 = (e - ol) * inv;
                tmin = fmaxf(tmin, fminf(t1, t2));
                tmax = fminf(tmax, fmaxf(t1, t2));
            }
            if (tmin <= tmax) {
                const int n = cnt < max_hits ? cnt : max_hits;
                int pos = n;
                while (pos > 0 && hit_t[(r * max_hits + pos - 1) * 2] > tmin) --pos;
                if (pos < max_hits) {
                    for (int k = (n < max_hits ? n : max_hits - 1); k > pos; --k) {
                        hit_t[(r * max_hits + k) * 2 + 0] = hit_t[(r * max_hits + k - 1) * 2 + 0];
                        hit_t[(r * max_hits + k) * 2 + 1] = hit_t[(r * max_hits + k - 1) * 2 + 1];
                        hit_box[r * max_hits + k] = hit_box[r * max_hits + k - 1];
                    }
                    hit_t[(r * max_hits + pos) * 2 + 0] = tmin;
                    hit_t[(r * max_hits + pos) * 2 + 1] = tmax;
                    hit_box[r * max_hits + pos] = m;
                }
                ++cnt;
            }
        }
        hit_count[r] = cnt;
    }
}

#define SETUP_MAXH 8
struct RaySetupArgs {
// ... 175 lines not shown
    PNR_REQUIRE(n_rays >= 0 && n_samples >= 1 && n_samples <= (1 << 26), "pnr_stratified_rng: bad size R=%lld N=%d", (long long)n_rays,
                n_samples);
    if (n_rays == 0) return PNR_OK;
    PNR_REQUIRE(rays && z_out, "pnr_stratified_rng: null pointer");
    const int64_t total = n_rays * n_samples;
    hipLaunchKernelGGL(k_stratified<PnrRngDev>, dim3(pnr_grid_cap((total + 255) / 256)), dim3(256), 0, (hipStream_t)stream,
                       rays, n_rays, n_samples, lindisp, (const float*)nullptr, z_out, rng);
    PNR_CHECK_LAUNCH("pnr_stratified_rng");
    return PNR_OK;
}

PNR_EXPORT int pnr_gen_rays(const float* intr4_host, const float* c2w12_host, int width, int height, float near_, float far_,
                            const int32_t* pix, int64_t n_rays, float* rays, void* stream)
{
    PNR_REQUIRE(intr4_host && c2w12_host, "pnr_gen_rays: null camera");
    PNR_REQUIRE(width >= 1 && height >= 1 && n_rays >= 0, "pnr_gen_rays: bad size");
    if (n_rays == 0) return PNR_OK;
    PNR_REQUIRE(pix || n_rays == (int64_t)width * height, "pnr_gen_rays: without pixel indices n_rays must be width*height");
    PNR_REQUIRE(intr4_host[0] != 0.0f && intr4_host[1] != 0.0f, "pnr_gen_rays: zero focal length");
    PNR_REQUIRE(rays && (((uintptr_t)rays) & 15) == 0, "pnr_gen_rays: rays must be a 16-byte aligned device buffer");
    GenRaysArgs a;
    a.fx = intr4_host[0]; a.fy = intr4_host[1]; a.cx = intr4_host[2]; a.cy = intr4_host[3];
    for (int k = 0; k < 12; ++k) a.c2w[k] = c2w12_host[k];
    a.width = width; a.near_ = near_; a.far_ = far_; a.pix = pix; a.R = n_rays; a.rays = rays;
    hipLaunchKernelGGL(k_gen_rays, dim3(pnr_grid_cap((n_rays + 255) / 256)), dim3(256), 0, (hipStream_t)stream, a);
    PNR_CHECK_LAUNCH("pnr_gen_rays");
    return PNR_OK;
}

PNR_EXPORT int pnr_points(const float* rays, const float* z, int64_t n_rays, int n_samples, float* pts_out,
                          void* stream)
{
    PNR_REQUIRE(n_rays >= 0 && n_samples >= 1, "pnr_points: bad size");
    if (n_rays == 0) return PNR_OK;
    PNR_REQUIRE(rays && z && pts_out, "pnr_points: null pointer");
    const int64_t total = n_rays * n_samples * 3;
    hipLaunchKernelGGL(k_points, dim3(pnr_grid_cap((total + 255) / 256)), dim3(256), 0, (hipStream_t)stream,
                       rays, z, n_rays, n_samples, pts_out);
    PNR_CHECK_LAUNCH("pnr_points");
    return PNR_OK;
}

PNR_EXPORT int pnr_embed(const float* x, int64_t n, int L, float* out, void* stream)
{
    PNR_REQUIRE(n >= 0 && L >= 0 && L <= 16, "pnr_embed: bad size n=%lld L=%d", (long long)n, L);
    if (n == 0) return PNR_OK;
    PNR_REQUIRE(x && out, "pnr_embed: null pointer");
    const int64_t total = n * (3 + 6 * L);
    hipLaunchKernelGGL(k_embed, dim3(pnr_grid_cap((total + 255) / 256)), dim3(256), 0, (hipStream_t)stream,
                       x, n, L, out);
    PNR_CHECK_LAUNCH("pnr_embed");
    return PNR_OK;
}

static void launch_sample_pdf_rng(const float* z, const float* weights, const PnrRngDev& rng, int64_t n_rays, int n_coarse, int n_fine,
                                  float* z_samples, int32_t* inds, float* z_fine, const PdfLabelArgs& lab, hipStream_t st)
{
    int P = 1;
    while (P < n_coarse + n_fine) P <<= 1;
    if (n_coarse <= 64 && P <= 256)
        hipLaunchKernelGGL(k_sample_pdf_rng, dim3(pnr_grid_cap(n_rays, 32)), dim3(64), 0, st, z, weights, n_rays, n_coarse, n_fine,
                           z_samples, inds, z_fine, lab, rng);
    else
        hipLaunchKernelGGL(k_sample_pdf_big_rng, dim3(pnr_grid_cap(n_rays, 32)), dim3(64), 0, st, z, weights, n_rays, n_coarse, n_fine,
                           z_samples, inds, z_fine, lab, rng);
}

static void launch_sample_pdf(const float* z, const float* weights, const float* u, int64_t n_rays, int n_coarse, int n_fine,
                              float* z_samples, int32_t* inds, float* z_fine, const PdfLabelArgs& lab, hipStream_t st)
{
    int P = 1;
    while (P < n_coarse + n_fine) P <<= 1;
    const bool general_only = getenv("PNR_SAMPLE_PDF_GENERAL") != nullptr;
    if (!u && !z_samples && !inds && z_fine && n_coarse <= 64 && n_fine <= 192 && P <= 256 && lab.max_hits <= 64 && !general_only)
        hipLaunchKernelGGL(k_sample_pdf_det, dim3(pnr_grid_cap(n_rays, 32)), dim3(64), 0, st, z, weights, n_rays, n_coarse, n_fine, z_fine, lab);
    else if (n_coarse <= 64 && P <= 256)
        hipLaunchKernelGGL(k_sample_pdf, dim3(pnr_grid_cap(n_rays, 32)), dim3(64), 0, st, z, weights, u, n_rays, n_coarse, n_fine,
                           z_samples, inds, z_fine, lab);
    else
        hipLaunchKernelGGL(k_sample_pdf_big, dim3(pnr_grid_cap(n_rays, 32)), dim3(64), 0, st, z, weights, u, n_rays, n_coarse,
                           n_fine, z_samples, inds, z_fine, lab);
}

PNR_EXPORT int pnr_sample_pdf(const float* z, const float* weights, const float* u, int64_t n_rays, int n_coarse,
                              int n_fine, float* z_samples, int32_t* inds, float* z_fine, void* stream)
{
    PNR_REQUIRE(n_rays <= 0 || (z && weights), "pnr_sample_pdf: null pointer");
    PNR_REQUIRE(n_coarse >= 3 && n_coarse <= PDF_MAXC, "pnr_sample_pdf: n_coarse=%d outside [3,%d]", n_coarse, PDF_MAXC);
    PNR_REQUIRE(n_fine >= 1 && n_coarse + n_fine <= PDF_MAXT, "pnr_sample_pdf: n_coarse+n_fine=%d > %d",
                n_coarse + n_fine, PDF_MAXT);
    if (n_rays <= 0) return PNR_OK;
    PdfLabelArgs lab;
    memset(&lab, 0, sizeof(lab));
    launch_sample_pdf(z, weights, u, n_rays, n_coarse, n_fine, z_samples, inds, z_fine, lab, (hipStream_t)stream);
    PNR_CHECK_LAUNCH("pnr_sample_pdf");
    return PNR_OK;
}

PNR_EXPORT int pnr_sample_pdf_rng(const float* z, const float* weights, const pnr_rng* rng_host, int64_t n_rays, int n_coarse,
                                  int n_fine, float* z_samples, int32_t* inds, float* z_fine, void* stream)
{
    PnrRngDev rng;
    const int rc = pnr_rng_check(rng_host, n_rays < 0 ? 0 : n_rays, "pnr_sample_pdf_rng", &rng);
    if (rc) return rc;
    PNR_REQUIRE(n_rays <= 0 || (z && weights), "pnr_sample_pdf_rng: null pointer");
    PNR_REQUIRE(n_coarse >= 3 && n_coarse <= PDF_MAXC, "pnr_sample_pdf_rng: n_coarse=%d outside [3,%d]", n_coarse, PDF_MAXC);
    PNR_REQUIRE(n_fine >= 1 && n_coarse + n_fine <= PDF_MAXT, "pnr_sample_pdf_rng: n_coarse+n_fine=%d > %d", n_coarse + n_fine, PDF_MAXT);
    if (n_rays <= 0) return PNR_OK;
    PdfLabelArgs lab;
    memset(&lab, 0, sizeof(lab));
    launch_sample_pdf_rng(z, weights, rng, n_rays, n_coarse, n_fine, z_samples, inds, z_fine, lab, (hipStream_t)stream);
    PNR_CHECK_LAUNCH("pnr_sample_pdf_rng");
    return PNR_OK;
}

PNR_EXPORT int pnr_sample_pdf_labels_rng(const float* z, const float* weights, const pnr_rng* rng_host, int64_t n_rays, int n_coarse,
                                         int n_fine, float* z_fine, const float* hit_t, const int32_t* hit_box, const int32_t* hit_count,
                                         int max_hits, const int32_t* box_ids, int32_t* label_sem, int32_t* label_inst, void* stream)
{
    PnrRngDev rng;
    const int rc = pnr_rng_check(rng_host, n_rays < 0 ? 0 : n_rays, "pnr_sample_pdf_labels_rng", &rng);
    if (rc) return rc;
    PNR_REQUIRE(n_rays <= 0 || (z && weights && z_fine), "pnr_sample_pdf_labels_rng: null pointer");
    PNR_REQUIRE(n_rays <= 0 || (hit_t && hit_box && hit_count && box_ids && label_sem && label_inst), "pnr_sample_pdf_labels_rng: null pointer");
    PNR_REQUIRE(n_coarse >= 3 && n_coarse <= PDF_MAXC, "pnr_sample_pdf_labels_rng: n_coarse=%d outside [3,%d]", n_coarse, PDF_MAXC);
    PNR_REQUIRE(n_fine >= 1 && n_coarse + n_fine <= PDF_MAXT, "pnr_sample_pdf_labels_rng: n_coarse+n_fine=%d > %d", n_coarse + n_fine,
                PDF_MAXT);
    PNR_REQUIRE(max_hits >= 1, "pnr_sample_pdf_labels_rng: bad max_hits");
    if (n_rays <= 0) return PNR_OK;
    PdfLabelArgs lab;
    lab.hit_t = hit_t; lab.hit_box = hit_box; lab.hit_count = hit_count; lab.max_hits = max_hits; lab.box_ids = box_ids;
    lab.label_sem = label_sem; lab.label_inst = label_inst;
    launch_sample_pdf_rng(z, weights, rng, n_rays, n_coarse, n_fine, nullptr, nullptr, z_fine, lab, (hipStream_t)stream);
    PNR_CHECK_LAUNCH("pnr_sample_pdf_labels_rng");
    return PNR_OK;
}

PNR_EXPORT int pnr_sample_pdf_labels(const float* z, const float* weights, const float* u, int64_t n_rays, int n_coarse, int n_fine,
                                     float* z_fine, const float* hit_t, const int32_t* hit_box, const int32_t* hit_count,
                                     int max_hits, const int32_t* box_ids, int32_t* label_sem, int32_t* label_inst, void* stream)
{
    PNR_REQUIRE(n_rays <= 0 || (z && weights && z_fine), "pnr_sample_pdf_labels: null pointer");
    PNR_REQUIRE(n_rays <= 0 || (hit_t && hit_box && hit_count && box_ids && label_sem && label_inst), "pnr_sample_pdf_labels: null pointer");
    PNR_REQUIRE(n_coarse >= 3 && n_coarse <= PDF_MAXC, "pnr_sample_pdf_labels: n_coarse=%d outside [3,%d]", n_coarse, PDF_MAXC);
    PNR_REQUIRE(n_fine >= 1 && n_coarse + n_fine <= PDF_MAXT, "pnr_sample_pdf_labels: n_coarse+n_fine=%d > %d", n_coarse + n_fine, PDF_MAXT);
    PNR_REQUIRE(max_hits >= 1, "pnr_sample_pdf_labels: bad max_hits");
    if (n_rays <= 0) return PNR_OK;
    PdfLabelArgs lab;
    lab.hit_t = hit_t; lab.hit_box = hit_box; lab.hit_count = hit_count; lab.max_hits = max_hits; lab.box_ids = box_ids;
    lab.label_sem = label_sem; lab.label_inst = label_inst;
    launch_sample_pdf(z, weights, u, n_rays, n_coarse, n_fine, nullptr, nullptr, z_fine, lab, (hipStream_t)stream);
    PNR_CHECK_LAUNCH("pnr_sample_pdf_labels");
    return PNR_OK;
}

static int ray_setup_impl(const float* rays, int64_t n_rays, const float* box, int n_box, int max_hits, const int32_t* box_ids,
                          int n_samples, int lindisp, const float* t_rand, const PnrRngDev* rng, int hull, float* hit_t, int32_t* hit_box,
                          int32_t* hit_count, float* z_out, int32_t* label_sem, int32_t* label_inst, void* stream);

PNR_EXPORT int pnr_ray_setup(const float* rays, int64_t n_rays, const float* box, int n_box, int max_hits, const int32_t* box_ids,
                             int n_samples, int lindisp, const float* t_rand, int hull, float* hit_t, int32_t* hit_box,
                             int32_t* hit_count, float* z_out, int32_t* label_sem, int32_t* label_inst, void* stream)
{
    return ray_setup_impl(rays, n_rays, box, n_box, max_hits, box_ids, n_samples, lindisp, t_rand, nullptr, hull, hit_t, hit_box, hit_count,
                          z_out, label_sem, label_inst, stream);
}
// ... 100 lines not shown
```

panopticnerf_amd/ops.py:

```python
import ctypes
import os

import torch

from . import _lib
from ._lib import MlpDesc, MlpParamsHost


def _stream():
    return ctypes.c_void_p(torch.cuda.current_stream().cuda_stream)


def _chk(t, name, dtype=torch.float32):
    if t is None:
        return None
    if not t.is_cuda:
        raise RuntimeError(f"{name}: expected a GPU tensor (the HIP path has no CPU fallback)")
    if t.dtype != dtype:
        raise TypeError(f"{name}: expected {dtype}, got {t.dtype}")
    if not t.is_contiguous():
        raise ValueError(f"{name}: tensor must be contiguous")
    return t


# ... 403 lines not shown


@_on_device
def composite(raw, z, rays, n_sem=0, n_inst=0, channel_major=True, noise=None, label_sem=None, label_inst=None,
              sem_mode=0, white_bkgd=False, want_weights=True, out=None):
    z, rays = _chk(z, "z"), _chk(rays, "rays")
    draw = noise if _draw(noise) else None
    noise = None if draw is not None else _chk(noise, "noise")
    label_sem = _chk(label_sem, "label_sem", torch.int32)
    label_inst = _chk(label_inst, "label_inst", torch.int32)
    R, N = z.shape
    ch = 4 + n_sem + n_inst
    if channel_major:
        ss, sc = 1, _chk_raw(raw, ch, R * N)
    else:
        _chk(raw, "raw")
        assert tuple(raw.shape) == (R, N, ch)
        ss, sc = ch, 1
    dev = z.device
    out = _maps(out, R, N, n_sem, n_inst, label_sem, label_inst, want_weights, dev)
    g = out.get
    if draw is not None:
        _lib.check(_lib.load().pnr_composite_rng(_p(raw), ss, sc, _p(z), _p(rays), ctypes.byref(draw.desc()), _p(label_sem),
                                                 _p(label_inst), R, N, n_sem, n_inst, int(sem_mode), int(bool(white_bkgd)),
                                                 _p(out["rgb"]), _p(out["depth"]), _p(out["acc"]), _p(g("weights")),
                                                 _p(g("semantic")), _p(g("instance")), _p(g("fix_semantic")),
                                                 _p(g("fix_instance")), _stream()), "pnr_composite_rng")
        return out
    _lib.check(_lib.load().pnr_composite(_p(raw), ss, sc, _p(z), _p(rays), _p(noise), _p(label_sem), _p(label_inst),
                                         R, N, n_sem, n_inst, int(sem_mode), int(bool(white_bkgd)),
                                         _p(out["rgb"]), _p(out["depth"]), _p(out["acc"]), _p(g("weights")),
                                         _p(g("semantic")), _p(g("instance")), _p(g("fix_semantic")),
                                         _p(g("fix_instance")), _stream()), "pnr_composite")
    return out


def _maps(out, R, N, n_sem, n_inst, label_sem, label_inst, want_weights, dev, drop=()):
    f32 = dict(device=dev, dtype=torch.float32)
    shapes = {"rgb": (R, 3), "depth": (R,), "acc": (R,)}
    if want_weights:
        shapes["weights"] = (R, N)
    if n_sem:
        shapes["semantic"] = (R, n_sem)
        if label_sem is not None:
            shapes["fix_semantic"] = (R, n_sem)
    if n_inst:
        shapes["instance"] = (R, n_inst)
        if label_inst is not None:
            shapes["fix_instance"] = (R, n_inst)
    for k in drop:
        shapes.pop(k, None)
    res = {}
    for k, shp in shapes.items():
        t = out.get(k) if out else None
        if t is None:
            t = torch.empty(shp, **f32)
        elif tuple(t.shape) != shp or t.dtype != torch.float32 or t.device != dev or not t.is_contiguous():
            raise ValueError("out[%r] must be a contiguous fp32 tensor of shape %s on %s" % (k, shp, dev))
        res[k] = t
    return res


def fused_supported(desc, n_samples, sem_mode=0, noise=None):
    ok = (desc.precision == _lib.PREC_BF16 and int(sem_mode) in (0, 1) and noise is None and n_samples % 32 == 0
          and 32 <= n_samples <= 256 and desc.n_sem + desc.n_inst <= 128)
    if ok and int(sem_mode) == 1 and desc.n_sem + desc.n_inst > 0:
        ok = int(_lib.load().pnr_mlp_fused_plan(ctypes.byref(desc_for_mode(desc, 1)))) >= 1
    return ok


def desc_for_mode(desc, sem_mode):
    want = _lib.MLP_SOFTMAX if int(sem_mode) == 1 else 0
    if (desc.flags & _lib.MLP_SOFTMAX) == want:
        return desc
    return _desc_with(desc, flags=(desc.flags & ~_lib.MLP_SOFTMAX) | want)


def fused_image(sem_mode=0):
    return "softmax" if int(sem_mode) == 1 else True


@_on_device
def mlp_forward_composite(desc, packed, rays, z, label_sem=None, label_inst=None, white_bkgd=False, want_weights=True, out=None,
                          sem_mode=0, wg_cap=0):
    rays, z, packed = _chk(rays, "rays"), _chk(z, "z"), _chk(packed, "packed", torch.uint8)
    label_sem = _chk(label_sem, "label_sem", torch.int32)
    label_inst = _chk(label_inst, "label_inst", torch.int32)
    R, N = z.shape
    n_sem, n_inst = desc.n_sem, desc.n_inst
    dev = z.device
    lib = _lib.load()
    desc = desc_for_mode(desc, sem_mode)
    if wg_cap:
        desc = _desc_with(desc, flags=(desc.flags & 0xFFFF) | ((int(wg_cap) & 0x1FF) << 16))
    nbytes = lib.pnr_mlp_forward_composite_workspace_bytes(ctypes.byref(desc), R, N, int(bool(want_weights)))
    if nbytes < 0:
        raise RuntimeError("pnr_mlp_forward_composite: unsupported geometry (n_samples=%d must be a multiple of 32)" % N)
    ws = torch.empty(int(nbytes), device=dev, dtype=torch.uint8)
    out = _maps(out, R, N, n_sem, n_inst, label_sem, label_inst, want_weights, dev)
    g = out.get
    _lib.check(lib.pnr_mlp_forward_composite(ctypes.byref(desc), _p(packed), _p(rays), _p(z), R, N, _p(label_sem), _p(label_inst),
                                             int(bool(white_bkgd)), _p(out["rgb"]), _p(out["depth"]), _p(out["acc"]),
                                             _p(g("weights")), _p(g("semantic")), _p(g("instance")), _p(g("fix_semantic")),
                                             _p(g("fix_instance")), _p(ws), _stream()), "pnr_mlp_forward_composite")
    return out


WEIGHTS_ONLY_DROPS = ("rgb", "semantic", "instance")


def sigma_pass_supported(desc, n_samples, noise=None):
    if not (desc.precision == _lib.PREC_BF16 and noise is None and n_samples % 32 == 0 and 32 <= n_samples <= 256
            and desc.n_sem + desc.n_inst <= 128):
        return False
    return int(_lib.load().pnr_mlp_packed_bytes(ctypes.byref(_desc_with(desc, plan=3)))) > 0


@_on_device
def mlp_forward_weights(desc, packed, rays, z, label_sem=None, label_inst=None, out=None):
    if desc.plan != 3:
        raise ValueError("mlp_forward_weights: needs the plan-3 image (net.packed(level, device, fused='sigma')), not plan %d" % desc.plan)
    rays, z, packed = _chk(rays, "rays"), _chk(z, "z"), _chk(packed, "packed", torch.uint8)
    label_sem = _chk(label_sem, "label_sem", torch.int32)
    label_inst = _chk(label_inst, "label_inst", torch.int32)
    R, N = z.shape
    dev = z.device
    lib = _lib.load()
    nbytes = lib.pnr_mlp_forward_composite_workspace_bytes(ctypes.byref(desc), R, N, 1)
    if nbytes < 0:
        raise RuntimeError("pnr_mlp_forward_composite: unsupported geometry (n_samples=%d must be a multiple of 32)" % N)
    ws = torch.empty(int(nbytes), device=dev, dtype=torch.uint8)
    out = _maps(out, R, N, desc.n_sem, desc.n_inst, label_sem, label_inst, True, dev, drop=WEIGHTS_ONLY_DROPS)
    g = out.get
    _lib.check(lib.pnr_mlp_forward_composite(ctypes.byref(desc), _p(packed), _p(rays), _p(z), R, N, _p(label_sem), _p(label_inst),
                                             0, None, _p(out["depth"]), _p(out["acc"]), _p(out["weights"]), None, None,
                                             _p(g("fix_semantic")), _p(g("fix_instance")), _p(ws), _stream()), "pnr_mlp_forward_composite")
    return out


QUERY_WANTS = ("sigma", "labels", "panoptic", "logits")


def field_query_supported(desc):
    return bool(_lib.load().pnr_mlp_query_supported(ctypes.byref(desc)))


def query_keys(desc, want):
    want = (want,) if isinstance(want, str) else tuple(want)
    bad = [w for w in want if w not in QUERY_WANTS]
    if bad:
        raise ValueError("query: unknown output %r in want (known: %s)" % (bad[0], ", ".join(QUERY_WANTS)))
    keys = []
    if "sigma" in want:
        keys.append("sigma")
    if "labels" in want:
        keys += (["sem_label"] if desc.n_sem else []) + (["inst_label"] if desc.n_inst else [])
    if "panoptic" in want and desc.n_sem:
        keys.append("panoptic")
    if "logits" in want:
        keys += (["sem_logits"] if desc.n_sem else []) + (["inst_logits"] if desc.n_inst else [])
    if not keys:
        raise ValueError("query: want=%r asks for nothing this network has (n_sem=%d, n_inst=%d)" % (want, desc.n_sem, desc.n_inst))
    return keys


@_on_device
def mlp_query(desc, packed, points, want=("sigma", "labels"), is_thing=None, out=None):
    if desc.plan != 4:
        raise ValueError("mlp_query: needs the plan-4 image (net.packed(level, device, fused='field')), not plan %d" % desc.plan)
    keys = query_keys(desc, want)
    points, packed = _chk(points, "points"), _chk(packed, "packed", torch.uint8)
    is_thing = _chk(is_thing, "is_thing", torch.int32)
    if points.dim() != 2 or points.shape[1] != 3:
        raise ValueError("mlp_query: points must be (P, 3), got %s" % (tuple(points.shape),))
    if is_thing is not None and (not desc.n_sem or is_thing.numel() != desc.n_sem):
        raise ValueError("mlp_query: is_thing must hold n_sem=%d entries of a network with a semantic head" % desc.n_sem)
    P, dev = points.shape[0], points.device
    out = dict(out) if out else {}
    res, stride = {}, P
    for k in keys:
        if k.endswith("_logits"):
            n = desc.n_sem if k == "sem_logits" else desc.n_inst
            t = out.get(k)
            if t is None:
                t = alloc_raw(n, P, dev)
            elif (not t.is_cuda or t.dtype != torch.float32 or tuple(t.shape) != (n, P) or (P > 0 and t.stride(1) != 1)
                  or (n > 1 and t.stride(0) < P)):
                raise ValueError("mlp_query: out[%r] must be a float32 GPU tensor of shape %s with unit point stride" % (k, (n, P)))
            res[k] = t
        else:
            res[k] = _own(out.get(k), (P,), torch.float32 if k == "sigma" else torch.int32, dev, "mlp_query: out[%r]" % k)
    lg = [res[k] for k in ("sem_logits", "inst_logits") if k in res]
    if lg:
        stride = lg[0].stride(0) if lg[0].shape[0] > 1 else max(P, lg[0].stride(0))
        if any((t.stride(0) if t.shape[0] > 1 else stride) != stride for t in lg):
            raise ValueError("mlp_query: sem_logits and inst_logits must share one channel stride")
    g = res.get
    _lib.check(_lib.load().pnr_mlp_query(ctypes.byref(desc), _p(packed), _p(points), P, _p(g("sigma")), _p(g("sem_label")),
                                         _p(g("inst_label")), _p(g("panoptic")), _p(is_thing), _p(g("sem_logits")),
                                         _p(g("inst_logits")), stride, _stream()), "pnr_mlp_query")
    return res


@_on_device
def composite_backward(raw, z, rays, n_sem, n_inst, grads, noise=None, label_sem=None, label_inst=None,
                       ce_sem=None, ce_inst=None, sem_mode=0):
    raw, z, rays = _chk(raw, "raw"), _chk(z, "z"), _chk(rays, "rays")
    draw = noise if _draw(noise) else None
    noise = None if draw is not None else _chk(noise, "noise")
    label_sem = _chk(label_sem, "label_sem", torch.int32)
    label_inst = _chk(label_inst, "label_inst", torch.int32)
    R, N = z.shape
    g = {k: _chk(v.contiguous().float(), "g_" + k) for k, v in grads.items() if v is not None}
    ce_sem = None if ce_sem is None else _chk(ce_sem.reshape(1).float().contiguous(), "ce_sem")
    ce_inst = None if ce_inst is None else _chk(ce_inst.reshape(1).float().contiguous(), "ce_inst")
    d_raw = torch.empty_like(raw)
    if draw is not None:
        _lib.check(_lib.load().pnr_composite_backward_rng(_p(raw), R * N, _p(z), _p(rays), ctypes.byref(draw.desc()), R, N, n_sem, n_inst,
                                                          int(sem_mode), _p(g.get("rgb")), _p(g.get("depth")), _p(g.get("acc")),
                                                          _p(g.get("semantic")), _p(g.get("instance")), _p(g.get("weights")),
# ... 186 lines not shown
```

panopticnerf_amd/renderer.py:

```python
import os

import torch

from . import ops


def _get(cfg, name, default):
    return getattr(cfg, name, default) if cfg is not None else default


CHUNK_QUANTUM = 1024


PREAMBLE_EARLY = os.environ.get("PNR_OVERLAP_PRE", "1") != "0"
CHUNK_TAIL = 8


def chunk_plan(n_rays, chunk_size):
    n_rays, chunk_size = int(n_rays), max(1, int(chunk_size))
    if n_rays <= 0:
        return []
    n = -(-n_rays // chunk_size)
    if n > 1 and n_rays - (n - 1) * chunk_size <= chunk_size // CHUNK_TAIL:
        n -= 1
    size = -(-n_rays // n)
    if n > 1 and chunk_size >= CHUNK_QUANTUM * CHUNK_TAIL:
        size = -(-size // CHUNK_QUANTUM) * CHUNK_QUANTUM
    out, s = [], 0
    while s < n_rays:
        e = min(n_rays, s + size)
        out.append((s, e))
        s = e
    return out


class Renderer:
    def __init__(self, net, cfg=None):
        self.net = net
        self.cfg = cfg
        self.N_samples = _get(cfg, "N_samples", 64)
        self.N_importance = _get(cfg, "N_importance", _get(cfg, "cascade_samples", 0))
        self.chunk_size = _get(cfg, "chunk_size", 65536)
        self.perturb = _get(cfg, "perturb", 0.0)
        self.raw_noise_std = _get(cfg, "raw_noise_std", 0.0)
        self.white_bkgd = _get(cfg, "white_bkgd", False)
        self.lindisp = _get(cfg, "lindisp", False)
        self.max_hits = _get(cfg, "max_hits", 8)
        self.sem_mode = {"none": 0, "logits": 0, "softmax": 1}[_get(cfg, "semantic_activation", "none")]
        self.keep_weights = _get(cfg, "keep_weights", True)
        self.fuse = bool(_get(cfg, "fuse_composite", os.environ.get("PNR_FUSE", "1") != "0"))
        self.strict_hits = bool(_get(cfg, "strict_hits", False))
        self.coarse_outputs = _get(cfg, "coarse_outputs", "all")
        if self.coarse_outputs not in ("all", "weights"):
            raise ValueError("cfg.coarse_outputs must be 'all' or 'weights', not %r" % (self.coarse_outputs,))
        if self.coarse_outputs == "weights" and self.N_importance <= 0:
            raise ValueError("cfg.coarse_outputs = 'weights' needs a fine level (N_importance > 0): without one the coarse maps are "
                             "the render's output")
        self.bbox_sampling = _get(cfg, "bbox_sampling", "none")
        if self.bbox_sampling not in ("none", "hull"):
            raise ValueError("cfg.bbox_sampling must be 'none' or 'hull', not %r" % (self.bbox_sampling,))
        self._overflow = None
        self.rng = _get(cfg, "rng", "torch")
        if self.rng not in ("torch", "device"):
            raise ValueError("cfg.rng must be 'torch' or 'device', not %r" % (self.rng,))
        self.rng_state = None
        if self.rng == "device":
            seed = _get(cfg, "rng_seed", None)
            seed = torch.initial_seed() if seed is None else int(seed)
            seed = (seed + 2 ** 63) % 2 ** 64 - 2 ** 63
            p0 = next(iter(net.parameters()), None)
            self.rng_state = torch.tensor([seed, 0], dtype=torch.int64, device=p0.device if p0 is not None else "cpu")
        self.frame_outputs = bool(_get(cfg, "frame_outputs", os.environ.get("PNR_FRAME_OUT", "1") != "0"))
        self.overlap_levels = bool(_get(cfg, "overlap_levels", os.environ.get("PNR_OVERLAP", "1") != "0"))
        self._side_streams = {}
        if self.N_importance > 0 and getattr(net, "nerf_1", None) is None and not getattr(net, "share_coarse_fine", False):
            raise ValueError("make_renderer: cfg asks for a fine pass (N_importance / cascade_samples = %d) but the network "
                             "was built without a fine NeRF -- build it with make_network(cfg) from the SAME cfg, or set "
                             "cfg.share_coarse_fine = True to evaluate one NeRF at both levels on purpose" % self.N_importance)

    def _preamble(self, rays, box, box_ids, t_rand, z_out):
        hits = lab0 = None
        hull = self.bbox_sampling == "hull"
        if box is not None and self.max_hits <= ops.RAY_SETUP_MAX_HITS:
            hits, z, ls0, li0 = ops.ray_setup(rays, box, box_ids, self.N_samples, self.max_hits, self.lindisp, t_rand, hull, out=z_out)
            lab0 = (ls0, li0)
        else:
            if box is not None:
                hits = ops.bbox_hits(rays, box, self.max_hits)
            rays_s = ops.restrict_rays(rays, hits[0], hits[2]) if (hits is not None and hull) else rays
            z = ops.stratified(rays_s, self.N_samples, self.lindisp, t_rand, out=z_out)
        return hits, z, lab0

    def render_rays(self, rays, box=None, box_ids=None, t_rand=None, u=None, train=False, grad=False, out=None, sched=None, rng=None):
        net, Nc, Nf = self.net, self.N_samples, self.N_importance
        n0 = net.nerf(0)
        C, K = n0.n_sem, n0.n_inst
        dev = rays.device
        ret = {}
        hits = lab0 = None
        if t_rand is None and self.perturb > 0 and train:
            t_rand = ops.Draw(rng[0], 1, rng[1]) if rng is not None else torch.rand((rays.shape[0], Nc), device=dev)
        own = (lambda key: out.get(key)) if (out and not grad) else (lambda key: None)
        if sched is not None and sched.get("pre") is not None:
            hits, z, lab0 = sched["pre"]
        else:
            hits, z, lab0 = self._preamble(rays, box, box_ids, t_rand, own("z_vals_0"))
        if hits is not None and self.strict_hits:
            over = torch.stack([(hits[2] > self.max_hits).sum(), hits[2].max()])
            self._overflow = over if self._overflow is None else torch.stack([self._overflow[0] + over[0],
                                                                              torch.maximum(self._overflow[1], over[1])])

        def level(lv, zz, labels=None):
            ls = li = None
            if labels is not None:
                ls, li = labels
            elif hits is not None:
                ls, li = ops.sample_labels(zz, hits[0], hits[1], hits[2], box_ids)
            noise = None
            if self.raw_noise_std > 0 and train:
                if rng is not None:
                    noise = ops.Draw(rng[0], 3 + lv, rng[1], self.raw_noise_std)
                else:
                    noise = torch.randn(zz.shape, device=dev) * self.raw_noise_std
            if grad:
                from . import train as _train
                res = _train.level_train(self, lv, rays, zz, ls, li, noise)
            elif lv == 0 and self.coarse_outputs == "weights":
                mine = {k: own(f"{k}_0") for k in ("depth", "acc", "weights", "fix_semantic", "fix_instance")}
                mine = {k: v for k, v in mine.items() if v is not None}
                if self.fuse and ops.sigma_pass_supported(n0.desc(net.precision), zz.shape[1], noise):
                    desc, img = net.packed(0, dev, fused="sigma")
                    res = ops.mlp_forward_weights(desc, img, rays, zz, ls, li, out=mine)
                else:
                    desc, img = net.packed(0, dev)
                    raw = ops.mlp_forward(desc, img, rays, zz, channel_major=True)
                    res = ops.composite(raw, zz, rays, C, K, True, noise, ls, li, self.sem_mode, self.white_bkgd, True, out=mine)
                    res = {k: v for k, v in res.items() if k not in ops.WEIGHTS_ONLY_DROPS}
            else:
                need_w = self.keep_weights or (lv == 0 and Nf > 0)
                mine = {k: own(f"{k}_{lv}") for k in ("rgb", "depth", "acc", "weights", "semantic", "instance", "fix_semantic", "fix_instance")}
                mine = {k: v for k, v in mine.items() if v is not None}
                if self.fuse and ops.fused_supported(net.nerf(lv).desc(net.precision), zz.shape[1], self.sem_mode, noise):
                    desc, img = net.packed(lv, dev, fused=ops.fused_image(self.sem_mode))
                    if sched is not None and lv == 0 and sched.get("wait") is not None:
                        torch.cuda.current_stream(dev).wait_event(sched["wait"])
                    res = ops.mlp_forward_composite(desc, img, rays, zz, ls, li, self.white_bkgd, need_w, out=mine, sem_mode=self.sem_mode,
                                                    wg_cap=0 if sched is None else sched["caps"][lv])
                else:
                    desc, img = net.packed(lv, dev)
                    raw = ops.mlp_forward(desc, img, rays, zz, channel_major=True)
                    res = ops.composite(raw, zz, rays, C, K, True, noise, ls, li, self.sem_mode, self.white_bkgd, need_w, out=mine)
            for k, v in res.items():
                ret[f"{k}_{lv}"] = v
            ret[f"z_vals_{lv}"] = zz
            return res

        o0 = level(0, z, lab0)
        if Nf > 0:
            if u is None and self.perturb > 0 and train:
                u = ops.Draw(rng[0], 2, rng[1]) if rng is not None else torch.rand((rays.shape[0], Nf), device=dev)
            w0 = o0["weights"].detach().contiguous()
            if hits is not None:
                z_fine, ls1, li1 = ops.sample_pdf_labels(z, w0, Nf, hits, box_ids, u, out=own("z_vals_1"))
                lab1 = (ls1, li1)
            else:
                z_fine, _, _ = ops.sample_pdf(z, w0, Nf, u, want_samples=False, out=own("z_vals_1"))
                lab1 = None
            if sched is not None:
                sched["pdf_done"] = torch.cuda.Event()
                sched["pdf_done"].record(torch.cuda.current_stream(dev))
                if sched.get("before_fine") is not None:
                    sched["before_fine"]()
            level(1, z_fine, lab1)
        return ret

    def _empty_outputs(self, lead, has_box, dev, grad=False):
        n0 = self.net.nerf(0)
        C, K = n0.n_sem, n0.n_inst
        ret = {}
        for lv, N in ((0, self.N_samples),) + (((1, self.N_samples + self.N_importance),) if self.N_importance > 0 else ()):
            need_w = self.keep_weights or (lv == 0 and self.N_importance > 0)
            drop = ops.WEIGHTS_ONLY_DROPS if (lv == 0 and not grad and self.coarse_outputs == "weights") else ()
            m = ops._maps(None, 0, N, C, K, True if has_box else None, True if has_box else None, need_w, dev, drop=drop)
            m["z_vals"] = torch.empty((0, N), device=dev, dtype=torch.float32)
            for k, v in m.items():
                ret[f"{k}_{lv}"] = v.reshape(*lead, *v.shape[1:])
        return ret

    def _overlap_caps(self, dev, plan, grad, train, has_box, t_rand, u):
        if (not self.overlap_levels or grad or train or len(plan) < 2 or not self.fuse or not self.frame_outputs or self.N_importance <= 0
                or self.strict_hits or t_rand is not None or u is not None or self.raw_noise_std > 0 and train
                or self.coarse_outputs == "weights" or torch.cuda.is_current_stream_capturing()):
            return None
        net, Nc, Nt = self.net, self.N_samples, self.N_samples + self.N_importance
        for lv, N in ((0, Nc), (1, Nt)):
            d = net.nerf(lv).desc(net.precision)
            if not ops.fused_supported(d, N, self.sem_mode, None) or net.packed(lv, dev, fused=ops.fused_image(self.sem_mode))[0].plan != 2:
                return None
        cus = torch.cuda.get_device_properties(dev).multi_processor_count
        cap_c = int(round(cus * Nc / float(Nc + Nt) / 8.0)) * 8
        cap_f = cus - cap_c
        if cus % 8 or cap_c < 8 or cap_f < 8 or abs((Nc / float(cap_c)) / (Nt / float(cap_f)) - 1.0) > 0.05:
            return None
        return cap_c, cap_f

    def _frame_maps(self, R, has_box, dev):
        n0 = self.net.nerf(0)
        C, K = n0.n_sem, n0.n_inst
        frame = {}
        for lv, N in ((0, self.N_samples), (1, self.N_samples + self.N_importance)):
            need_w = self.keep_weights or lv == 0
            m = ops._maps(None, R, N, C, K, True if has_box else None, True if has_box else None, need_w, dev)
            m["z_vals"] = torch.empty((R, N), device=dev, dtype=torch.float32)
            for k, v in m.items():
                frame[f"{k}_{lv}"] = v
        return frame

    def _render_overlapped(self, rays, box, box_ids, plan, caps, lead):
        dev = rays.device
        R = rays.shape[0]
        cap_c, cap_f = caps
        frame = self._frame_maps(R, box is not None, dev)
        main = torch.cuda.current_stream(dev)
        if dev not in self._side_streams:
            self._side_streams[dev] = (torch.cuda.Stream(dev), torch.cuda.Stream(dev))
        side = self._side_streams[dev]
        start = torch.cuda.Event()
        start.record(main)
        for st in side:
            st.wait_event(start)
        prev_pdf = None
        pre = {}

        def preamble(cj):
            sj, ej = plan[cj]
            pre[cj] = self._preamble(rays[sj:ej], box, box_ids, None, frame["z_vals_0"][sj:ej])
        for ci, (s, e) in enumerate(plan):
            sched = {"wait": prev_pdf, "caps": (0 if ci == 0 else cap_c, 0 if ci == len(plan) - 1 else cap_f), "pdf_done": None,
                     "pre": pre.pop(ci, None),
                     "before_fine": (lambda cj=ci + 2: preamble(cj)) if (PREAMBLE_EARLY and ci + 2 < len(plan)) else None}
            with torch.cuda.stream(side[ci & 1]):
                o = self.render_rays(rays[s:e], box, box_ids, None, None, False, False, out={k: v[s:e] for k, v in frame.items()}, sched=sched)
                for k, v in o.items():
                    if v.data_ptr() != frame[k][s:e].data_ptr():
                        frame[k][s:e].copy_(v)
            prev_pdf = sched["pdf_done"]
        for st in side:
            done = torch.cuda.Event()
            done.record(st)
            main.wait_event(done)
# ... 107 lines not shown
```

Measured before the change: 1177.

## Fuse coarse compositing combine with PDF fine sampling into one tail kernel

Adds a deferred-combine flag so the coarse fused MLP pass skips its separate combine kernel. A new coarse-tail kernel then does the per-ray compositing and the inverse-CDF fine sampling (plus label lookup) together, keeping the weights on chip instead of writing them out and reading them back in a separate sample_pdf launch. It is on by default for inference with 64 coarse samples. In exchange it adds a specialized kernel path with size limits and duplicated sampling logic.

Measured after the change: 1176. No clear change (-0.0%).

```diff
diff --git a/include/pnr.h b/include/pnr.h
--- a/include/pnr.h
+++ b/include/pnr.h
@@ -41,6 +41,7 @@
 
 #define PNR_MLP_SOFTMAX 1
 #define PNR_MLP_WG_CAP(n) (((n) & 0x1FF) << 16)
+#define PNR_MLP_DEFER_COMBINE 4
 #define PNR_MLP_TRACE 0x7A00
 
 typedef struct pnr_mlp_params_host {
@@ -78,6 +79,12 @@
 int pnr_composite_combine(const pnr_mlp_desc* desc, const void* workspace, const float* z, int64_t n_rays, int n_samples,
                           const int32_t* label_sem, const int32_t* label_inst, int white_bkgd, float* rgb, float* depth,
                           float* acc, float* weights, float* sem, float* inst, float* fix_sem, float* fix_inst, void* stream);
+
+int pnr_coarse_tail(const pnr_mlp_desc* desc, const void* workspace, const float* z, int64_t n_rays, int n_coarse, int n_fine,
+                    const int32_t* label_sem, const int32_t* label_inst, int white_bkgd, float* rgb, float* depth, float* acc,
+                    float* weights, float* sem, float* inst, float* fix_sem, float* fix_inst, const float* hit_t,
+                    const int32_t* hit_box, const int32_t* hit_count, int max_hits, const int32_t* box_ids, float* z_fine,
+                    int32_t* label_sem_fine, int32_t* label_inst_fine, void* stream);
 
 int pnr_mlp_query(const pnr_mlp_desc* desc, const void* packed, const float* points, int64_t n_points,
                   float* sigma, int32_t* sem_label, int32_t* inst_label, int32_t* panoptic, const int32_t* is_thing,
diff --git a/panopticnerf_amd/_lib.py b/panopticnerf_amd/_lib.py
--- a/panopticnerf_amd/_lib.py
+++ b/panopticnerf_amd/_lib.py
@@ -9,7 +9,7 @@
 c_int = ctypes.c_int
 
 PREC_BF16, PREC_FP32 = 0, 1
-MLP_SOFTMAX, MLP_TRACE = 1, 0x7A00
+MLP_SOFTMAX, MLP_DEFER_COMBINE, MLP_TRACE = 1, 4, 0x7A00
 CAMERA_PINHOLE, CAMERA_FISHEYE = 0, 1
 
 
@@ -116,6 +116,8 @@
     "pnr_mlp_query_supported": (c_int, [ctypes.POINTER(MlpDesc)]),
     "pnr_composite_combine": (c_int, [ctypes.POINTER(MlpDesc), c_f, c_f, c_i64, c_int, c_f, c_f, c_int,
                                       c_f, c_f, c_f, c_f, c_f, c_f, c_f, c_f, c_f]),
+    "pnr_coarse_tail": (c_int, [ctypes.POINTER(MlpDesc), c_f, c_f, c_i64, c_int, c_int, c_f, c_f, c_int,
+                                c_f, c_f, c_f, c_f, c_f, c_f, c_f, c_f, c_f, c_f, c_f, c_int, c_f, c_f, c_f, c_f, c_f]),
 }
 
 _lib = None
diff --git a/panopticnerf_amd/csrc/pnr_combine_ray.h b/panopticnerf_amd/csrc/pnr_combine_ray.h
--- /dev/null
+++ b/panopticnerf_amd/csrc/pnr_combine_ray.h
@@ -0,0 +1,101 @@
+#pragma once
+#include "pnr_common.h"
+#include "pnr_fuse_record.h"
+#include "pnr_lane_ops.h"
+
+struct CombineArgs {
+    const float* rec; int rec_floats; const float4* ps; const float* z; const int32_t* lab_s; const int32_t* lab_i;
+    int64_t R; int N, C, K, white_bkgd;
+    float *rgb, *depth, *acc, *weights, *sem, *inst, *fix_sem, *fix_inst;
+};
+
+template <bool LOGITS, int NJ>
+__device__ __forceinline__ void combine_ray(const CombineArgs& a, int64_t ray, int lane, uint32_t* hist, float& w0, float& z0)
+{
+    constexpr int NT = 2 * NJ;
+    const int N = a.N, T = N >> 5, RF = a.rec_floats, C = a.C, K = a.K, CK = C + K;
+    const float* __restrict__ rec = a.rec + ray * T * RF;
+    const float4* __restrict__ ps = a.ps + ray * N;
+    const float* __restrict__ zr = a.z + ray * N;
+    const bool want_s = a.lab_s && a.fix_sem && C, want_i = a.lab_i && a.fix_inst && K;
+    const int32_t* __restrict__ lsr = want_s ? a.lab_s + ray * N : nullptr;
+    const int32_t* __restrict__ lir = want_i ? a.lab_i + ray * N : nullptr;
+    float q[NT];
+#pragma unroll
+    for (int k = 0; k < NT; ++k) q[k] = k < T ? rec[k * RF] : 1.0f;
+    float4 pv[NJ];
+    float zv[NJ];
+    int lsv[NJ], liv[NJ];
+#pragma unroll
+    for (int j = 0; j < NJ; ++j) {
+        const int i = lane + 64 * j;
+        const bool in = i < N;
+        pv[j] = in ? ps[i] : float4{0.0f, 0.0f, 0.0f, 0.0f};
+        zv[j] = in ? zr[i] : 0.0f;
+        lsv[j] = (in && want_s) ? lsr[i] : -1;
+        liv[j] = (in && want_i) ? lir[i] : -1;
+    }
+    float lg[2][NT];
+#pragma unroll
+    for (int h = 0; h < 2; ++h)
+#pragma unroll
+        for (int k = 0; k < NT; ++k) lg[h][k] = (LOGITS && k < T && lane + 64 * h < CK) ? rec[k * RF + PNR_FUSE_REC_LOGITS + lane + 64 * h] : 0.0f;
+    float Tk[NT];
+    float t = 1.0f;
+#pragma unroll
+    for (int k = 0; k < NT; ++k) {
+        Tk[k] = t;
+        if (k < T) t *= q[k];
+    }
+    if (want_s || want_i)
+        for (int c = lane; c < CK; c += 64) hist[c] = 0;
+    float r5[5] = {0.0f, 0.0f, 0.0f, 0.0f, 0.0f};
+    w0 = 0.0f;
+    z0 = zv[0];
+#pragma unroll
+    for (int j = 0; j < NJ; ++j) {
+        const int i = lane + 64 * j;
+        if (i < N) {
+            const float4 p = pv[j];
+            float tk = Tk[0];
+#pragma unroll
+            for (int k = 1; k < NT; ++k) tk = (i >> 5) == k ? Tk[k] : tk;
+            const float w = tk * p.x;
+            if (j == 0) w0 = w;
+            r5[0] += w;
+            r5[1] = fmaf(w, zv[j], r5[1]);
+            r5[2] = fmaf(w, 1.0f / (1.0f + expf(-p.y)), r5[2]);
+            r5[3] = fmaf(w, 1.0f / (1.0f + expf(-p.z)), r5[3]);
+            r5[4] = fmaf(w, 1.0f / (1.0f + expf(-p.w)), r5[4]);
+            if (a.weights) a.weights[ray * N + i] = w;
+            if (want_s || want_i) {
+                const uint32_t fx = (uint32_t)(w * PNR_FUSE_FIX_SCALE + 0.5f);
+                if (want_s) { const int l = lsv[j]; if (l >= 0 && l < C) atomicAdd(&hist[l], fx); }
+                if (want_i) { const int l = liv[j]; if (l >= 0 && l < K) atomicAdd(&hist[C + l], fx); }
+            }
+        }
+    }
+    group_sum_batch<64, 5>(r5);
+    if (lane == 0) {
+        if (a.acc) a.acc[ray] = r5[0];
+        if (a.depth) a.depth[ray] = r5[1];
+    }
+    if (lane < 3 && a.rgb) {
+        const float v = lane == 0 ? r5[2] : lane == 1 ? r5[3] : r5[4];
+        a.rgb[ray * 3 + lane] = a.white_bkgd ? v + (1.0f - r5[0]) : v;
+    }
+#pragma unroll
+    for (int h = 0; h < 2; ++h) {
+        const int c = lane + 64 * h;
+        if (c >= CK) continue;
+        if constexpr (LOGITS) {
+            float v = 0.0f;
+#pragma unroll
+            for (int k = 0; k < NT; ++k) if (k < T) v = fmaf(Tk[k], lg[h][k], v);
+            if (c < C) { if (a.sem) a.sem[ray * C + c] = v; }
+            else if (a.inst) a.inst[ray * K + (c - C)] = v;
+        }
+        if (c < C) { if (want_s) a.fix_sem[ray * C + c] = (float)hist[c] * (1.0f / PNR_FUSE_FIX_SCALE); }
+        else if (want_i) a.fix_inst[ray * K + (c - C)] = (float)hist[c] * (1.0f / PNR_FUSE_FIX_SCALE);
+    }
+}
diff --git a/panopticnerf_amd/csrc/pnr_composite.hip b/panopticnerf_amd/csrc/pnr_composite.hip
--- a/panopticnerf_amd/csrc/pnr_composite.hip
+++ b/panopticnerf_amd/csrc/pnr_composite.hip
@@ -1,5 +1,6 @@
 #include <stdlib.h>
 
+#include "pnr_combine_ray.h"
 #include "pnr_common.h"
 #include "pnr_fuse_record.h"
 #include "pnr_lane_ops.h"
@@ -553,12 +554,6 @@
 }
 
 
-struct CombineArgs {
-    const float* rec; int rec_floats; const float4* ps; const float* z; const int32_t* lab_s; const int32_t* lab_i;
-    int64_t R; int N, C, K, white_bkgd;
-    float *rgb, *depth, *acc, *weights, *sem, *inst, *fix_sem, *fix_inst;
-};
-
 template <bool LOGITS>
 __global__ __launch_bounds__(256) void k_composite_combine(CombineArgs a)
 {
@@ -566,89 +561,8 @@
     const int lane = threadIdx.x & 63, wv = threadIdx.x >> 6;
     const int64_t ray = ((int64_t)blockIdx.x * blockDim.x + threadIdx.x) >> 6;
     if (ray >= a.R) return;
-    const int N = a.N, T = N >> 5, RF = a.rec_floats, C = a.C, K = a.K, CK = C + K;
-    const float* __restrict__ rec = a.rec + ray * T * RF;
-    const float4* __restrict__ ps = a.ps + ray * N;
-    const float* __restrict__ zr = a.z + ray * N;
-    const bool want_s = a.lab_s && a.fix_sem && C, want_i = a.lab_i && a.fix_inst && K;
-    const int32_t* __restrict__ lsr = want_s ? a.lab_s + ray * N : nullptr;
-    const int32_t* __restrict__ lir = want_i ? a.lab_i + ray * N : nullptr;
-    float q[8];
-#pragma unroll
-    for (int k = 0; k < 8; ++k) q[k] = k < T ? rec[k * RF] : 1.0f;
-    float4 pv[4];
-    float zv[4];
-    int lsv[4], liv[4];
-#pragma unroll
-    for (int j = 0; j < 4; ++j) {
-        const int i = lane + 64 * j;
-        const bool in = i < N;
-        pv[j] = in ? ps[i] : float4{0.0f, 0.0f, 0.0f, 0.0f};
-        zv[j] = in ? zr[i] : 0.0f;
-        lsv[j] = (in && want_s) ? lsr[i] : -1;
-        liv[j] = (in && want_i) ? lir[i] : -1;
-    }
-    float lg[2][8];
-#pragma unroll
-    for (int h = 0; h < 2; ++h)
-#pragma unroll
-        for (int k = 0; k < 8; ++k) lg[h][k] = (LOGITS && k < T && lane + 64 * h < CK) ? rec[k * RF + PNR_FUSE_REC_LOGITS + lane + 64 * h] : 0.0f;
-    float Tk[8];
-    float t = 1.0f;
-#pragma unroll
-    for (int k = 0; k < 8; ++k) {
-        Tk[k] = t;
-        if (k < T) t *= q[k];
-    }
-    uint32_t* hist = hist_all[wv];
-    if (want_s || want_i)
-        for (int c = lane; c < CK; c += 64) hist[c] = 0;
-    float r5[5] = {0.0f, 0.0f, 0.0f, 0.0f, 0.0f};
-#pragma unroll
-    for (int j = 0; j < 4; ++j) {
-        const int i = lane + 64 * j;
-        if (i < N) {
-            const float4 p = pv[j];
-            float tk = Tk[0];
-#pragma unroll
-            for (int k = 1; k < 8; ++k) tk = (i >> 5) == k ? Tk[k] : tk;
-            const float w = tk * p.x;
-            r5[0] += w;
-            r5[1] = fmaf(w, zv[j], r5[1]);
-            r5[2] = fmaf(w, 1.0f / (1.0f + expf(-p.y)), r5[2]);
-            r5[3] = fmaf(w, 1.0f / (1.0f + expf(-p.z)), r5[3]);
-            r5[4] = fmaf(w, 1.0f / (1.0f + expf(-p.w)), r5[4]);
-            if (a.weights) a.weights[ray * N + i] = w;
-            if (want_s || want_i) {
-                const uint32_t fx = (uint32_t)(w * PNR_FUSE_FIX_SCALE + 0.5f);
-                if (want_s) { const int l = lsv[j]; if (l >= 0 && l < C) atomicAdd(&hist[l], fx); }
-                if (want_i) { const int l = liv[j]; if (l >= 0 && l < K) atomicAdd(&hist[C + l], fx); }
-            }
-        }
-    }
-    group_sum_batch<64, 5>(r5);
-    if (lane == 0) {
-        if (a.acc) a.acc[ray] = r5[0];
-        if (a.depth) a.depth[ray] = r5[1];
-    }
-    if (lane < 3 && a.rgb) {
-        const float v = lane == 0 ? r5[2] : lane == 1 ? r5[3] : r5[4];
-        a.rgb[ray * 3 + lane] = a.white_bkgd ? v + (1.0f - r5[0]) : v;
-    }
-#pragma unroll
-    for (int h = 0; h < 2; ++h) {
-        const int c = lane + 64 * h;
-        if (c >= CK) continue;
-        if constexpr (LOGITS) {
-            float v = 0.0f;
-#pragma unroll
-            for (int k = 0; k < 8; ++k) if (k < T) v = fmaf(Tk[k], lg[h][k], v);
-            if (c < C) { if (a.sem) a.sem[ray * C + c] = v; }
-            else if (a.inst) a.inst[ray * K + (c - C)] = v;
-        }
-        if (c < C) { if (want_s) a.fix_sem[ray * C + c] = (float)hist[c] * (1.0f / PNR_FUSE_FIX_SCALE); }
-        else if (want_i) a.fix_inst[ray * K + (c - C)] = (float)hist[c] * (1.0f / PNR_FUSE_FIX_SCALE);
-    }
+    float w0, z0;
+    combine_ray<LOGITS, 4>(a, ray, lane, hist_all[wv], w0, z0);
 }
 
 int pnr_composite_combine_launch(const float* rec, int rec_floats, bool logit_sums, const float4* ps, const float* z,
diff --git a/panopticnerf_amd/csrc/pnr_mlp.hip b/panopticnerf_amd/csrc/pnr_mlp.hip
--- a/panopticnerf_amd/csrc/pnr_mlp.hip
+++ b/panopticnerf_amd/csrc/pnr_mlp.hip
@@ -824,6 +824,11 @@
                                  const int32_t* label_sem, const int32_t* label_inst, int64_t R, int N, int C, int K, int white_bkgd,
                                  float* rgb, float* depth, float* acc, float* weights, float* sem, float* inst, float* fix_sem,
                                  float* fix_inst, hipStream_t st);
+int pnr_coarse_tail_launch(const float* rec, int rec_floats, bool logit_sums, const float4* ps, const float* z, const int32_t* label_sem,
+                           const int32_t* label_inst, int64_t R, int N, int C, int K, int white_bkgd, float* rgb, float* depth, float* acc,
+                           float* weights, float* sem, float* inst, float* fix_sem, float* fix_inst, int n_fine, float* z_fine,
+                           const float* hit_t, const int32_t* hit_box, const int32_t* hit_count, int max_hits, const int32_t* box_ids,
+                           int32_t* label_sem_fine, int32_t* label_inst_fine, hipStream_t st);
 
 static int record_floats(const pnr_mlp_desc& d)
 {
@@ -939,6 +944,7 @@
     PNR_REQUIRE((!fix_sem || label_sem) && (!fix_inst || label_inst), "pnr_composite_combine: fix_* outputs need their labels");
     PNR_REQUIRE(desc->plan != 3 || (!rgb && !sem && !inst), "pnr_composite_combine: a plan-3 (sigma-only) workspace has no rgb, semantic "
                 "or instance maps: pass null for them");
+    if (desc->flags & PNR_MLP_DEFER_COMBINE) return PNR_OK;
     const int rf = record_floats(*desc);
     const int64_t tiles = (n_rays * n_samples + 255) / 256 * 8;
     const float* rec = (const float*)workspace;
@@ -960,9 +966,37 @@
     MlpArgs a;
     int rc = fused_mlp_launch(desc, packed, rays, z, n_rays, n_samples, workspace, stream, a);
     if (rc != PNR_OK) return rc;
+    if (desc->flags & PNR_MLP_DEFER_COMBINE) return PNR_OK;
     return pnr_composite_combine_launch(a.rec, a.rec_floats, desc->plan != 3, a.ps, z, fix_sem ? label_sem : nullptr, fix_inst ? label_inst : nullptr,
                                         n_rays, n_samples, desc->n_sem, desc->n_inst, white_bkgd, rgb, depth, acc, weights, sem, inst,
                                         fix_sem, fix_inst, (hipStream_t)stream);
+}
+
+PNR_EXPORT int pnr_coarse_tail(const pnr_mlp_desc* desc, const void* workspace, const float* z, int64_t n_rays, int n_coarse, int n_fine,
+                               const int32_t* label_sem, const int32_t* label_inst, int white_bkgd, float* rgb, float* depth, float* acc,
+                               float* weights, float* sem, float* inst, float* fix_sem, float* fix_inst, const float* hit_t,
+                               const int32_t* hit_box, const int32_t* hit_count, int max_hits, const int32_t* box_ids, float* z_fine,
+                               int32_t* label_sem_fine, int32_t* label_inst_fine, void* stream)
+{
+    int rc = pnr_mlp_validate(desc);
+    if (rc != PNR_OK) return rc;
+    PNR_REQUIRE(n_rays >= 0, "pnr_coarse_tail: bad size");
+    PNR_REQUIRE(desc->precision == PNR_PREC_BF16 && desc->plan != 4, "pnr_coarse_tail: needs the workspace of a bf16 fused compositing pass "
+                "(plan 0..3)");
+    PNR_REQUIRE(desc->n_sem + desc->n_inst <= 128, "pnr_coarse_tail: n_sem + n_inst <= 128");
+    PNR_REQUIRE((!fix_sem || label_sem) && (!fix_inst || label_inst), "pnr_coarse_tail: fix_* outputs need their labels");
+    PNR_REQUIRE(desc->plan != 3 || (!rgb && !sem && !inst), "pnr_coarse_tail: a plan-3 (sigma-only) workspace has no rgb, semantic or "
+                "instance maps: pass null for them");
+    PNR_REQUIRE(n_rays * (int64_t)(n_coarse > 0 ? n_coarse : 0) < ((int64_t)1 << 31) - 4096, "pnr_coarse_tail: R*N exceeds 2^31");
+    if (n_rays == 0) return PNR_OK;
+    PNR_REQUIRE(workspace && (((uintptr_t)workspace) & 15) == 0, "pnr_coarse_tail: workspace must be a 16-byte aligned device buffer");
+    const int rf = record_floats(*desc);
+    const int64_t tiles = (n_rays * (int64_t)n_coarse + 255) / 256 * 8;
+    const float* rec = (const float*)workspace;
+    return pnr_coarse_tail_launch(rec, rf, desc->plan != 3, (const float4*)(rec + tiles * rf), z, fix_sem ? label_sem : nullptr,
+                                  fix_inst ? label_inst : nullptr, n_rays, n_coarse, desc->n_sem, desc->n_inst, white_bkgd, rgb, depth,
+                                  acc, weights, sem, inst, fix_sem, fix_inst, n_fine, z_fine, hit_t, hit_box, hit_count, max_hits, box_ids,
+                                  label_sem_fine, label_inst_fine, (hipStream_t)stream);
 }
 
 PNR_EXPORT int pnr_mlp_forward_train(const pnr_mlp_desc* desc, const void* packed, const float* rays, const float* z,
diff --git a/panopticnerf_amd/csrc/pnr_mlp_pack.cpp b/panopticnerf_amd/csrc/pnr_mlp_pack.cpp
--- a/panopticnerf_amd/csrc/pnr_mlp_pack.cpp
+++ b/panopticnerf_amd/csrc/pnr_mlp_pack.cpp
@@ -32,7 +32,7 @@
                 (d->plan == 3 && pnr_plan3_supported(*d)) || (d->plan == 4 && pnr_plan4_supported(*d)),
                 "pnr_mlp: plan=%d is not available for this geometry (ask pnr_mlp_fused_plan; plans 3 and 4: bf16 only)", d->plan);
     const uint32_t trace = (uint32_t)d->flags & 0xFF00u;
-    PNR_REQUIRE(((uint32_t)d->flags & ~(uint32_t)(PNR_MLP_SOFTMAX | 0xFF70u | PNR_MLP_WG_CAP(0x1FF))) == 0 && (trace == 0 || trace == PNR_MLP_TRACE) &&
+    PNR_REQUIRE(((uint32_t)d->flags & ~(uint32_t)(PNR_MLP_SOFTMAX | PNR_MLP_DEFER_COMBINE | 0xFF70u | PNR_MLP_WG_CAP(0x1FF))) == 0 && (trace == 0 || trace == PNR_MLP_TRACE) &&
                 (trace != 0 || ((uint32_t)d->flags & 0x70u) == 0),
                 "pnr_mlp: unknown bits in flags=0x%x (zero-initialise pnr_mlp_desc; PNR_MLP_* are the defined bits)", (unsigned)d->flags);
     PNR_REQUIRE(((uint32_t)d->clk_probe[0] & 15u) == 0, "pnr_mlp: clk_probe=0x%08x%08x is not a 16-byte aligned device address "
diff --git a/panopticnerf_amd/csrc/pnr_sampling.hip b/panopticnerf_amd/csrc/pnr_sampling.hip
--- a/panopticnerf_amd/csrc/pnr_sampling.hip
+++ b/panopticnerf_amd/csrc/pnr_sampling.hip
@@ -1,3 +1,4 @@
+#include "pnr_combine_ray.h"
 #include "pnr_common.h"
 #include "pnr_philox.h"
 #include <stdlib.h>
@@ -325,175 +326,232 @@
 #define PDF_DET_WPE 8
 #endif
 #if PDF_DET_WPE
-__attribute__((amdgpu_waves_per_eu(PDF_DET_WPE, PDF_DET_WPE)))
+#define PDF_DET_OCCUPANCY __attribute__((amdgpu_waves_per_eu(PDF_DET_WPE, PDF_DET_WPE)))
+#else
+#define PDF_DET_OCCUPANCY
 #endif
+
+#ifndef COARSE_TAIL_WPE
+#define COARSE_TAIL_WPE PDF_DET_WPE
+#endif
+#if COARSE_TAIL_WPE
+#define COARSE_TAIL_OCCUPANCY __attribute__((amdgpu_waves_per_eu(COARSE_TAIL_WPE, COARSE_TAIL_WPE)))
+#else
+#define COARSE_TAIL_OCCUPANCY
+#endif
+
+struct PdfDetLds {
+    float z[64], w[64], pdf[64], cdf[64], bins[64];
+    float zs[192], out[256];
+    float total, part[32];
+};
+struct PdfDetHits { int cnt, ls, li; float ti, to; };
+
+__device__ __forceinline__ PdfDetHits pdf_det_hits(const PdfLabelArgs& lab, int64_t r, int lane)
+{
+    PdfDetHits h;
+    h.cnt = 0; h.ls = -1; h.li = -1; h.ti = 0.0f; h.to = 0.0f;
+    if (lab.label_sem) {
+        const int mh = lab.max_hits;
+        const int c0 = lab.hit_count[r];
+        h.cnt = c0 < mh ? c0 : mh;
+        if (lane < h.cnt) {
+            const float2 t2 = *reinterpret_cast<const float2*>(lab.hit_t + (r * mh + lane) * 2);
+            h.ti = t2.x; h.to = t2.y;
+            const int m = lab.hit_box[r * mh + lane];
+            h.ls = lab.box_ids[m * 2];
+            h.li = lab.box_ids[m * 2 + 1];
+        }
+    }
+    return h;
+}
+
+__device__ __forceinline__ void pdf_det_ray(PdfDetLds& s, const float zl, const float wl, const PdfDetHits hits, int64_t r, int Nc, int Nf,
+                                            int topc, int topf, float* __restrict__ zfine_out, const PdfLabelArgs& lab, int lane)
+{
+    const int nb = Nc - 1, nw = Nc - 2, Nt = Nc + Nf;
+    const int cnt = hits.cnt, h_ls = hits.ls, h_li = hits.li;
+    const float h_ti = hits.ti, h_to = hits.to;
+    float* const s_z = s.z; float* const s_w = s.w; float* const s_pdf = s.pdf; float* const s_cdf = s.cdf; float* const s_bins = s.bins;
+    float* const s_zs = s.zs; float* const s_out = s.out; float* const s_part = s.part;
+    s_z[lane] = zl;
+    s_w[lane] = wl;
+    const float zn = __shfl_down(zl, 1, 64), wn = __shfl_down(wl, 1, 64);
+    s_bins[lane] = 0.5f * (zn + zl);
+    __syncthreads();
+    if (lane < 32) {
+        const int k = lane >> 3, l = lane & 7, nv = nw / 8, groups = nv / 4;
+        float pacc = 0.0f;
+        for (int g = 0; g < groups; ++g) pacc = pacc + (s_w[(g * 4 + k) * 8 + l + 1] + 1e-5f);
+        if (k == 0)
+            for (int v = groups * 4; v < nv; ++v) pacc = pacc + (s_w[v * 8 + l + 1] + 1e-5f);
+        s_part[lane] = pacc;
+    }
+    __syncthreads();
+    if (lane == 0) {
+        const int nv = nw / 8;
+        float total = 0.0f;
+        for (int j = nv * 8; j < nw; ++j) total = total + (s_w[j + 1] + 1e-5f);
+        for (int l = 0; l < 8; ++l) {
+            float p0 = s_part[l];
+            p0 = p0 + s_part[8 + l]; p0 = p0 + s_part[16 + l]; p0 = p0 + s_part[24 + l];
+            total = total + p0;
+        }
+        s.total = total;
+    }
+    __syncthreads();
+    const float total = s.total;
+    const float pl = lane < nw ? (wn + 1e-5f) / total : 0.0f;
+    s_pdf[lane] = pl;
+    double c = (double)pl;
+    bool exact = __all(pl == 0.0f || pl >= 0x1p-28f);
+    if (exact) {
+#pragma unroll
+        for (int d = 1; d < 64; d <<= 1) {
+            const double o = __shfl_up(c, d, 64);
+            if (lane >= d) c += o;
+        }
+        exact = __shfl(c, 63, 64) < 1.999;
+    }
+    if (exact) {
+        if (lane == 0) s_cdf[0] = 0.0f;
+        if (lane < nw) s_cdf[lane + 1] = (float)c;
+    } else {
+        __syncthreads();
+        if (lane == 0) {
+            double cc = 0.0;
+            s_cdf[0] = 0.0f;
+            for (int j = 0; j < nw; ++j) {
+                cc += (double)s_pdf[j];
+                s_cdf[j + 1] = (float)cc;
+            }
+        }
+    }
+    __syncthreads();
+    bool asc = lane + 1 >= Nc || zl <= zn;
+    for (int i = lane; i < Nf; i += 64) {
+        const float uu = pnr_linspace01(i, Nf);
+        int pos = 0;
+        for (int st = topc; st >= 1; st >>= 1) {
+            const int p = pos + st, q = p <= nb ? p : nb;
+            pos = (p <= nb && s_cdf[q - 1] <= uu) ? p : pos;
+        }
+        const int inds = pos;
+        const int below = inds - 1 > 0 ? inds - 1 : 0;
+        const int above = inds < nb - 1 ? inds : nb - 1;
+        const float cb = s_cdf[below];
+        float denom = s_cdf[above] - cb;
+        if (denom < 1e-5f) denom = 1.0f;
+        const float t = (uu - cb) / denom;
+        const float bb = s_bins[below];
+        const float span = s_bins[above] - bb;
+        const float m = t * span;
+        const float zs = bb + m;
+        s_zs[i] = zs;
+    }
+    __syncthreads();
+    for (int i = lane; i + 1 < Nf; i += 64) asc = asc && (s_zs[i] <= s_zs[i + 1]);
+    if (__all(asc)) {
+        if (lane < Nc) {
+            int pos = 0;
+            for (int st = topf; st >= 1; st >>= 1) {
+                const int p = pos + st, q = p <= Nf ? p : Nf;
+                pos = (p <= Nf && s_zs[q - 1] < zl) ? p : pos;
+            }
+            s_out[lane + pos] = zl;
+        }
+        for (int j = lane; j < Nf; j += 64) {
+            const float v = s_zs[j];
+            int pos = 0;
+            for (int st = topc; st >= 1; st >>= 1) {
+                const int p = pos + st, q = p <= Nc ? p : Nc;
+                pos = (p <= Nc && s_z[q - 1] <= v) ? p : pos;
+            }
+            s_out[j + pos] = v;
+        }
+        __syncthreads();
+    } else {
+        int P = 1;
+        while (P < Nt) P <<= 1;
+        pdf_bitonic_fallback(s_out, s_z, s_zs, Nc, Nf, P, lane);
+    }
+    float* __restrict__ zo = zfine_out + r * Nt;
+    for (int i0 = 0; i0 < Nt; i0 += 256) {
+        float zz[4];
+        int best[4], ls[4], li[4];
+        float bt[4];
+#pragma unroll
+        for (int k = 0; k < 4; ++k) {
+            const int i = i0 + lane + 64 * k;
+            zz[k] = i < Nt ? s_out[i < Nt ? i : 0] : 0.0f;
+            best[k] = -1; ls[k] = -1; li[k] = -1; bt[k] = 0.0f;
+            if (i < Nt) zo[i] = zz[k];
+        }
+        if (lab.label_sem) {
+            for (int h = 0; h < cnt; ++h) {
+                const float ti = __int_as_float(__builtin_amdgcn_readlane(__float_as_int(h_ti), h));
+                const float to = __int_as_float(__builtin_amdgcn_readlane(__float_as_int(h_to), h));
+                const int hs = __builtin_amdgcn_readlane(h_ls, h), hi2 = __builtin_amdgcn_readlane(h_li, h);
+#pragma unroll
+                for (int k = 0; k < 4; ++k) {
+                    const bool take = ti <= zz[k] && zz[k] <= to && (best[k] < 0 || ti < bt[k]);
+                    best[k] = take ? h : best[k];
+                    bt[k] = take ? ti : bt[k];
+                    ls[k] = take ? hs : ls[k];
+                    li[k] = take ? hi2 : li[k];
+                }
+            }
+#pragma unroll
+            for (int k = 0; k < 4; ++k) {
+                const int i = i0 + lane + 64 * k;
+                if (i < Nt) {
+                    lab.label_sem[r * Nt + i] = ls[k];
+                    lab.label_inst[r * Nt + i] = li[k];
+                }
+            }
+        }
+    }
+    __syncthreads();
+}
+
+__device__ __forceinline__ void pdf_det_strides(int Nc, int Nf, int& topc, int& topf)
+{
+    topc = topf = 1;
+    while (topc * 2 <= Nc) topc *= 2;
+    while (topf * 2 <= Nf) topf *= 2;
+}
+
+PDF_DET_OCCUPANCY
 __global__ __launch_bounds__(64) void k_sample_pdf_det(const float* __restrict__ z, const float* __restrict__ weights, int64_t R, int Nc,
                                                         int Nf, float* __restrict__ zfine_out, const PdfLabelArgs lab)
 {
-    __shared__ float s_z[64], s_w[64], s_pdf[64], s_cdf[64], s_bins[64];
-    __shared__ float s_zs[192], s_out[256];
-    __shared__ float s_total, s_part[32];
+    __shared__ PdfDetLds s;
     const int lane = threadIdx.x;
-    const int nb = Nc - 1, nw = Nc - 2, Nt = Nc + Nf;
-    int topc = 1, topf = 1;
-    while (topc * 2 <= Nc) topc *= 2;
-    while (topf * 2 <= Nf) topf *= 2;
-    const int mh = lab.max_hits;
+    int topc, topf;
+    pdf_det_strides(Nc, Nf, topc, topf);
     for (int64_t r = blockIdx.x; r < R; r += gridDim.x) {
         const float* __restrict__ zr = z + r * Nc;
         const float* __restrict__ wr = weights + r * Nc;
         const float zl = lane < Nc ? zr[lane] : 0.0f, wl = lane < Nc ? wr[lane] : 0.0f;
-        int cnt = 0, h_ls = -1, h_li = -1;
-        float h_ti = 0.0f, h_to = 0.0f;
-        if (lab.label_sem) {
-            const int c0 = lab.hit_count[r];
-            cnt = c0 < mh ? c0 : mh;
-            if (lane < cnt) {
-                const float2 t2 = *reinterpret_cast<const float2*>(lab.hit_t + (r * mh + lane) * 2);
-                h_ti = t2.x; h_to = t2.y;
-                const int m = lab.hit_box[r * mh + lane];
-                h_ls = lab.box_ids[m * 2];
-                h_li = lab.box_ids[m * 2 + 1];
-            }
-        }
-        s_z[lane] = zl;
-        s_w[lane] = wl;
-        const float zn = __shfl_down(zl, 1, 64), wn = __shfl_down(wl, 1, 64);
-        s_bins[lane] = 0.5f * (zn + zl);
-        __syncthreads();
-        if (lane < 32) {
-            const int k = lane >> 3, l = lane & 7, nv = nw / 8, groups = nv / 4;
-            float pacc = 0.0f;
-            for (int g = 0; g < groups; ++g) pacc = pacc + (s_w[(g * 4 + k) * 8 + l + 1] + 1e-5f);
-            if (k == 0)
-                for (int v = groups * 4; v < nv; ++v) pacc = pacc + (s_w[v * 8 + l + 1] + 1e-5f);
-            s_part[lane] = pacc;
-        }
-        __syncthreads();
-        if (lane == 0) {
-            const int nv = nw / 8;
-            float total = 0.0f;
-            for (int j = nv * 8; j < nw; ++j) total = total + (s_w[j + 1] + 1e-5f);
-            for (int l = 0; l < 8; ++l) {
-                float p0 = s_part[l];
-                p0 = p0 + s_part[8 + l]; p0 = p0 + s_part[16 + l]; p0 = p0 + s_part[24 + l];
-                total = total + p0;
-            }
-            s_total = total;
-        }
-        __syncthreads();
-        const float total = s_total;
-        const float pl = lane < nw ? (wn + 1e-5f) / total : 0.0f;
-        s_pdf[lane] = pl;
-        double c = (double)pl;
-        bool exact = __all(pl == 0.0f || pl >= 0x1p-28f);
-        if (exact) {
-#pragma unroll
-            for (int d = 1; d < 64; d <<= 1) {
-                const double o = __shfl_up(c, d, 64);
-                if (lane >= d) c += o;
-            }
-            exact = __shfl(c, 63, 64) < 1.999;
-        }
-        if (exact) {
-            if (lane == 0) s_cdf[0] = 0.0f;
-            if (lane < nw) s_cdf[lane + 1] = (float)c;
-        } else {
-            __syncthreads();
-            if (lane == 0) {
-                double cc = 0.0;
-                s_cdf[0] = 0.0f;
-                for (int j = 0; j < nw; ++j) {
-                    cc += (double)s_pdf[j];
-                    s_cdf[j + 1] = (float)cc;
-                }
-            }
-        }
-        __syncthreads();
-        bool asc = lane + 1 >= Nc || zl <= zn;
-        for (int i = lane; i < Nf; i += 64) {
-            const float uu = pnr_linspace01(i, Nf);
-            int pos = 0;
-            for (int st = topc; st >= 1; st >>= 1) {
-                const int p = pos + st, q = p <= nb ? p : nb;
-                pos = (p <= nb && s_cdf[q - 1] <= uu) ? p : pos;
-            }
-            const int inds = pos;
-            const int below = inds - 1 > 0 ? inds - 1 : 0;
-            const int above = inds < nb - 1 ? inds : nb - 1;
-            const float cb = s_cdf[below];
-            float denom = s_cdf[above] - cb;
-            if (denom < 1e-5f) denom = 1.0f;
-            const float t = (uu - cb) / denom;
-            const float bb = s_bins[below];
-            const float span = s_bins[above] - bb;
-            const float m = t * span;
-            const float zs = bb + m;
-            s_zs[i] = zs;
-        }
-        __syncthreads();
-        for (int i = lane; i + 1 < Nf; i += 64) asc = asc && (s_zs[i] <= s_zs[i + 1]);
-        if (__all(asc)) {
-            if (lane < Nc) {
-                int pos = 0;
-                for (int st = topf; st >= 1; st >>= 1) {
-                    const int p = pos + st, q = p <= Nf ? p : Nf;
-                    pos = (p <= Nf && s_zs[q - 1] < zl) ? p : pos;
-                }
-                s_out[lane + pos] = zl;
-            }
-            for (int j = lane; j < Nf; j += 64) {
-                const float v = s_zs[j];
-                int pos = 0;
-                for (int st = topc; st >= 1; st >>= 1) {
-                    const int p = pos + st, q = p <= Nc ? p : Nc;
-                    pos = (p <= Nc && s_z[q - 1] <= v) ? p : pos;
-                }
-                s_out[j + pos] = v;
-            }
-            __syncthreads();
-        } else {
-            int P = 1;
-            while (P < Nt) P <<= 1;
-            pdf_bitonic_fallback(s_out, s_z, s_zs, Nc, Nf, P, lane);
-        }
-        float* __restrict__ zo = zfine_out + r * Nt;
-        for (int i0 = 0; i0 < Nt; i0 += 256) {
-            float zz[4];
-            int best[4], ls[4], li[4];
-            float bt[4];
-#pragma unroll
-            for (int k = 0; k < 4; ++k) {
-                const int i = i0 + lane + 64 * k;
-                zz[k] = i < Nt ? s_out[i < Nt ? i : 0] : 0.0f;
-                best[k] = -1; ls[k] = -1; li[k] = -1; bt[k] = 0.0f;
-                if (i < Nt) zo[i] = zz[k];
-            }
-            if (lab.label_sem) {
-                for (int h = 0; h < cnt; ++h) {
-                    const float ti = __int_as_float(__builtin_amdgcn_readlane(__float_as_int(h_ti), h));
-                    const float to = __int_as_float(__builtin_amdgcn_readlane(__float_as_int(h_to), h));
-                    const int hs = __builtin_amdgcn_readlane(h_ls, h), hi2 = __builtin_amdgcn_readlane(h_li, h);
-#pragma unroll
-                    for (int k = 0; k < 4; ++k) {
-                        const bool take = ti <= zz[k] && zz[k] <= to && (best[k] < 0 || ti < bt[k]);
-                        best[k] = take ? h : best[k];
-                        bt[k] = take ? ti : bt[k];
-                        ls[k] = take ? hs : ls[k];
-                        li[k] = take ? hi2 : li[k];
-                    }
-                }
-#pragma unroll
-                for (int k = 0; k < 4; ++k) {
-                    const int i = i0 + lane + 64 * k;
-                    if (i < Nt) {
-                        lab.label_sem[r * Nt + i] = ls[k];
-                        lab.label_inst[r * Nt + i] = li[k];
-                    }
-                }
-            }
-        }
-        __syncthreads();
+        const PdfDetHits hits = pdf_det_hits(lab, r, lane);
+        pdf_det_ray(s, zl, wl, hits, r, Nc, Nf, topc, topf, zfine_out, lab, lane);
+    }
+}
+
+template <bool LOGITS>
+COARSE_TAIL_OCCUPANCY
+__global__ __launch_bounds__(64) void k_coarse_tail(const CombineArgs a, int Nf, float* __restrict__ zfine_out, const PdfLabelArgs lab)
+{
+    __shared__ PdfDetLds s;
+    __shared__ uint32_t hist[128];
+    const int lane = threadIdx.x;
+    int topc, topf;
+    pdf_det_strides(a.N, Nf, topc, topf);
+    for (int64_t r = blockIdx.x; r < a.R; r += gridDim.x) {
+        const PdfDetHits hits = pdf_det_hits(lab, r, lane);
+        float wl, zl;
+        combine_ray<LOGITS, 1>(a, r, lane, hist, wl, zl);
+        pdf_det_ray(s, zl, wl, hits, r, a.N, Nf, topc, topf, zfine_out, lab, lane);
     }
 }
 
@@ -835,6 +893,40 @@
                            n_fine, z_samples, inds, z_fine, lab);
 }
 
+int pnr_coarse_tail_launch(const float* rec, int rec_floats, bool logit_sums, const float4* ps, const float* z, const int32_t* label_sem,
+                           const int32_t* label_inst, int64_t R, int N, int C, int K, int white_bkgd, float* rgb, float* depth, float* acc,
+                           float* weights, float* sem, float* inst, float* fix_sem, float* fix_inst, int n_fine, float* z_fine,
+                           const float* hit_t, const int32_t* hit_box, const int32_t* hit_count, int max_hits, const int32_t* box_ids,
+                           int32_t* label_sem_fine, int32_t* label_inst_fine, hipStream_t st)
+{
+    PNR_REQUIRE(N == 64, "pnr_coarse_tail: n_coarse=%d: the fused tail takes 64 coarse samples (use pnr_composite_combine + pnr_sample_pdf)", N);
+    PNR_REQUIRE(n_fine >= 1 && n_fine <= 192, "pnr_coarse_tail: n_fine=%d outside [1,192] (use pnr_composite_combine + pnr_sample_pdf)", n_fine);
+    PNR_REQUIRE(C >= 0 && K >= 0 && C + K <= 128, "pnr_coarse_tail: n_sem + n_inst <= 128");
+    PNR_REQUIRE(rec && ps && z && z_fine, "pnr_coarse_tail: null pointer");
+    PNR_REQUIRE(getenv("PNR_SAMPLE_PDF_GENERAL") == nullptr, "pnr_coarse_tail: PNR_SAMPLE_PDF_GENERAL asks for the general sample_pdf body "
+                "(use pnr_composite_combine + pnr_sample_pdf)");
+    PdfLabelArgs lab;
+    memset(&lab, 0, sizeof(lab));
+    if (label_sem_fine || label_inst_fine || hit_t || hit_box || hit_count) {
+        PNR_REQUIRE(hit_t && hit_box && hit_count && box_ids && label_sem_fine && label_inst_fine,
+                    "pnr_coarse_tail: the fine labels need hit_t, hit_box, hit_count, box_ids and both label outputs");
+        PNR_REQUIRE(max_hits >= 1 && max_hits <= 64, "pnr_coarse_tail: max_hits=%d outside [1,64] (use pnr_composite_combine + "
+                    "pnr_sample_pdf_labels)", max_hits);
+        PNR_REQUIRE((((uintptr_t)hit_t) & 7) == 0, "pnr_coarse_tail: hit_t must be 8-byte aligned");
+        lab.hit_t = hit_t; lab.hit_box = hit_box; lab.hit_count = hit_count; lab.max_hits = max_hits; lab.box_ids = box_ids;
+        lab.label_sem = label_sem_fine; lab.label_inst = label_inst_fine;
+    }
+    CombineArgs a;
+    a.rec = rec; a.rec_floats = rec_floats; a.ps = ps; a.z = z; a.lab_s = label_sem; a.lab_i = label_inst;
+    a.R = R; a.N = N; a.C = C; a.K = K; a.white_bkgd = white_bkgd;
+    a.rgb = rgb; a.depth = depth; a.acc = acc; a.weights = weights; a.sem = sem; a.inst = inst; a.fix_sem = fix_sem; a.fix_inst = fix_inst;
+    const dim3 grid(pnr_grid_cap(R, 32));
+    if (logit_sums) hipLaunchKernelGGL(k_coarse_tail<true>, grid, dim3(64), 0, st, a, n_fine, z_fine, lab);
+    else hipLaunchKernelGGL(k_coarse_tail<false>, grid, dim3(64), 0, st, a, n_fine, z_fine, lab);
+    PNR_CHECK_LAUNCH("pnr_coarse_tail");
+    return PNR_OK;
+}
+
 PNR_EXPORT int pnr_sample_pdf(const float* z, const float* weights, const float* u, int64_t n_rays, int n_coarse,
                               int n_fine, float* z_samples, int32_t* inds, float* z_fine, void* stream)
 {
diff --git a/panopticnerf_amd/ops.py b/panopticnerf_amd/ops.py
--- a/panopticnerf_amd/ops.py
+++ b/panopticnerf_amd/ops.py
@@ -509,7 +509,7 @@
 
 @_on_device
 def mlp_forward_composite(desc, packed, rays, z, label_sem=None, label_inst=None, white_bkgd=False, want_weights=True, out=None,
-                          sem_mode=0, wg_cap=0):
+                          sem_mode=0, wg_cap=0, defer_combine=False):
     rays, z, packed = _chk(rays, "rays"), _chk(z, "z"), _chk(packed, "packed", torch.uint8)
     label_sem = _chk(label_sem, "label_sem", torch.int32)
     label_inst = _chk(label_inst, "label_inst", torch.int32)
@@ -520,6 +520,8 @@
     desc = desc_for_mode(desc, sem_mode)
     if wg_cap:
         desc = _desc_with(desc, flags=(desc.flags & 0xFFFF) | ((int(wg_cap) & 0x1FF) << 16))
+    if defer_combine:
+        desc = _desc_with(desc, flags=desc.flags | _lib.MLP_DEFER_COMBINE)
     nbytes = lib.pnr_mlp_forward_composite_workspace_bytes(ctypes.byref(desc), R, N, int(bool(want_weights)))
     if nbytes < 0:
         raise RuntimeError("pnr_mlp_forward_composite: unsupported geometry (n_samples=%d must be a multiple of 32)" % N)
@@ -530,7 +532,7 @@
                                              int(bool(white_bkgd)), _p(out["rgb"]), _p(out["depth"]), _p(out["acc"]),
                                              _p(g("weights")), _p(g("semantic")), _p(g("instance")), _p(g("fix_semantic")),
                                              _p(g("fix_instance")), _p(ws), _stream()), "pnr_mlp_forward_composite")
-    return out
+    return (out, (desc, ws)) if defer_combine else out
 
 
 WEIGHTS_ONLY_DROPS = ("rgb", "semantic", "instance")
@@ -544,7 +546,7 @@
 
 
 @_on_device
-def mlp_forward_weights(desc, packed, rays, z, label_sem=None, label_inst=None, out=None):
+def mlp_forward_weights(desc, packed, rays, z, label_sem=None, label_inst=None, out=None, defer_combine=False):
     if desc.plan != 3:
         raise ValueError("mlp_forward_weights: needs the plan-3 image (net.packed(level, device, fused='sigma')), not plan %d" % desc.plan)
     rays, z, packed = _chk(rays, "rays"), _chk(z, "z"), _chk(packed, "packed", torch.uint8)
@@ -553,6 +555,8 @@
     R, N = z.shape
     dev = z.device
     lib = _lib.load()
+    if defer_combine:
+        desc = _desc_with(desc, flags=desc.flags | _lib.MLP_DEFER_COMBINE)
     nbytes = lib.pnr_mlp_forward_composite_workspace_bytes(ctypes.byref(desc), R, N, 1)
     if nbytes < 0:
         raise RuntimeError("pnr_mlp_forward_composite: unsupported geometry (n_samples=%d must be a multiple of 32)" % N)
@@ -562,7 +566,44 @@
     _lib.check(lib.pnr_mlp_forward_composite(ctypes.byref(desc), _p(packed), _p(rays), _p(z), R, N, _p(label_sem), _p(label_inst),
                                              0, None, _p(out["depth"]), _p(out["acc"]), _p(out["weights"]), None, None,
                                              _p(g("fix_semantic")), _p(g("fix_instance")), _p(ws), _stream()), "pnr_mlp_forward_composite")
-    return out
+    return (out, (desc, ws)) if defer_combine else out
+
+
+COARSE_TAIL_NC, COARSE_TAIL_MAX_NF, COARSE_TAIL_MAX_HITS = 64, 192, 64
+
+
+def coarse_tail_supported(n_coarse, n_fine, u=None, max_hits=None, want_samples=False):
+    return (int(n_coarse) == COARSE_TAIL_NC and 1 <= int(n_fine) <= COARSE_TAIL_MAX_NF and u is None and not want_samples
+            and (max_hits is None or 1 <= int(max_hits) <= COARSE_TAIL_MAX_HITS) and os.environ.get("PNR_SAMPLE_PDF_GENERAL") is None)
+
+
+@_on_device
+def coarse_tail(pending, z, n_importance, maps, label_sem=None, label_inst=None, white_bkgd=False, hits=None, box_ids=None, out=None):
+    desc, ws = pending
+    z = _chk(z, "z")
+    label_sem = _chk(label_sem, "label_sem", torch.int32)
+    label_inst = _chk(label_inst, "label_inst", torch.int32)
+    R, Nc = z.shape
+    dev = z.device
+    Nt = Nc + int(n_importance)
+    z_fine = _own(out, (R, Nt), torch.float32, dev, "coarse_tail")
+    hit_t = hit_box = hit_count = ls = li = None
+    max_hits = 0
+    if hits is not None:
+        hit_t, hit_box, hit_count = _chk(hits[0], "hit_t"), _chk(hits[1], "hit_box", torch.int32), _chk(hits[2], "hit_count", torch.int32)
+        box_ids = _chk(box_ids, "box_ids", torch.int32)
+        max_hits = hit_box.shape[1]
+        ls = torch.empty((R, Nt), device=dev, dtype=torch.int32)
+        li = torch.empty((R, Nt), device=dev, dtype=torch.int32)
+    else:
+        box_ids = None
+    g = maps.get
+    _lib.check(_lib.load().pnr_coarse_tail(ctypes.byref(desc), _p(ws), _p(z), R, Nc, int(n_importance), _p(label_sem), _p(label_inst),
+                                           int(bool(white_bkgd)), _p(g("rgb")), _p(g("depth")), _p(g("acc")), _p(g("weights")),
+                                           _p(g("semantic")), _p(g("instance")), _p(g("fix_semantic")), _p(g("fix_instance")),
+                                           _p(hit_t), _p(hit_box), _p(hit_count), int(max_hits), _p(box_ids), _p(z_fine), _p(ls), _p(li),
+                                           _stream()), "pnr_coarse_tail")
+    return z_fine, ls, li
 
 
 QUERY_WANTS = ("sigma", "labels", "panoptic", "logits")
diff --git a/panopticnerf_amd/renderer.py b/panopticnerf_amd/renderer.py
--- a/panopticnerf_amd/renderer.py
+++ b/panopticnerf_amd/renderer.py
@@ -73,6 +73,8 @@
         self.frame_outputs = bool(_get(cfg, "frame_outputs", os.environ.get("PNR_FRAME_OUT", "1") != "0"))
         self.overlap_levels = bool(_get(cfg, "overlap_levels", os.environ.get("PNR_OVERLAP", "1") != "0"))
         self._side_streams = {}
+        self.coarse_tail = bool(_get(cfg, "coarse_tail", os.environ.get("PNR_COARSE_TAIL", "1") != "0"))
+        self.tail_launches = 0
         if self.N_importance > 0 and getattr(net, "nerf_1", None) is None and not getattr(net, "share_coarse_fine", False):
             raise ValueError("make_renderer: cfg asks for a fine pass (N_importance / cascade_samples = %d) but the network "
                              "was built without a fine NeRF -- build it with make_network(cfg) from the SAME cfg, or set "
@@ -110,12 +112,17 @@
             self._overflow = over if self._overflow is None else torch.stack([self._overflow[0] + over[0],
                                                                               torch.maximum(self._overflow[1], over[1])])
 
+        want_tail = (self.coarse_tail and not grad and Nf > 0 and u is None and not (self.perturb > 0 and train)
+                     and ops.coarse_tail_supported(Nc, Nf, None, None if hits is None else self.max_hits))
+        tail = {}
+
         def level(lv, zz, labels=None):
             ls = li = None
             if labels is not None:
                 ls, li = labels
             elif hits is not None:
                 ls, li = ops.sample_labels(zz, hits[0], hits[1], hits[2], box_ids)
+            defer = want_tail and lv == 0
             noise = None
             if self.raw_noise_std > 0 and train:
                 if rng is not None:
@@ -130,7 +137,10 @@
                 mine = {k: v for k, v in mine.items() if v is not None}
                 if self.fuse and ops.sigma_pass_supported(n0.desc(net.precision), zz.shape[1], noise):
                     desc, img = net.packed(0, dev, fused="sigma")
-                    res = ops.mlp_forward_weights(desc, img, rays, zz, ls, li, out=mine)
+                    res = ops.mlp_forward_weights(desc, img, rays, zz, ls, li, out=mine, defer_combine=defer)
+                    if defer:
+                        res, pending = res
+                        tail.update(pending=pending, maps=res, labels=(ls, li), white_bkgd=False)
                 else:
                     desc, img = net.packed(0, dev)
                     raw = ops.mlp_forward(desc, img, rays, zz, channel_major=True)
@@ -145,7 +155,10 @@
                     if sched is not None and lv == 0 and sched.get("wait") is not None:
                         torch.cuda.current_stream(dev).wait_event(sched["wait"])
                     res = ops.mlp_forward_composite(desc, img, rays, zz, ls, li, self.white_bkgd, need_w, out=mine, sem_mode=self.sem_mode,
-                                                    wg_cap=0 if sched is None else sched["caps"][lv])
+                                                    wg_cap=0 if sched is None else sched["caps"][lv], defer_combine=defer)
+                    if defer:
+                        res, pending = res
+                        tail.update(pending=pending, maps=res, labels=(ls, li), white_bkgd=self.white_bkgd)
                 else:
                     desc, img = net.packed(lv, dev)
                     raw = ops.mlp_forward(desc, img, rays, zz, channel_major=True)
@@ -159,13 +172,19 @@
         if Nf > 0:
             if u is None and self.perturb > 0 and train:
                 u = ops.Draw(rng[0], 2, rng[1]) if rng is not None else torch.rand((rays.shape[0], Nf), device=dev)
-            w0 = o0["weights"].detach().contiguous()
-            if hits is not None:
-                z_fine, ls1, li1 = ops.sample_pdf_labels(z, w0, Nf, hits, box_ids, u, out=own("z_vals_1"))
-                lab1 = (ls1, li1)
+            if tail:
+                z_fine, ls1, li1 = ops.coarse_tail(tail["pending"], z, Nf, tail["maps"], tail["labels"][0], tail["labels"][1],
+                                                   tail["white_bkgd"], hits, box_ids, out=own("z_vals_1"))
+                lab1 = (ls1, li1) if hits is not None else None
+                self.tail_launches += 1
             else:
-                z_fine, _, _ = ops.sample_pdf(z, w0, Nf, u, want_samples=False, out=own("z_vals_1"))
-                lab1 = None
+                w0 = o0["weights"].detach().contiguous()
+                if hits is not None:
+                    z_fine, ls1, li1 = ops.sample_pdf_labels(z, w0, Nf, hits, box_ids, u, out=own("z_vals_1"))
+                    lab1 = (ls1, li1)
+                else:
+                    z_fine, _, _ = ops.sample_pdf(z, w0, Nf, u, want_samples=False, out=own("z_vals_1"))
+                    lab1 = None
             if sched is not None:
                 sched["pdf_done"] = torch.cuda.Event()
                 sched["pdf_done"].record(torch.cuda.current_stream(dev))
```
